# nipponjo/tts-arabic-pytorch

Measured on AMD Instinct MI355X. Metric: audio samples/sec (FastPitch+HiFi-GAN, synthetic 64-phoneme inputs), higher is better.
Workload: dtype f32

## Files before the change

include/ttsamd.h:

```cpp
#ifndef TTSAMD_H
#define TTSAMD_H

#include <stdint.h>

#ifdef __cplusplus
extern "C" {
#endif

#define TTSAMD_OK 0
#define TTSAMD_EINVAL (-1)
#define TTSAMD_EHIP (-2)
#define TTSAMD_ENOMEM (-3)

typedef struct ttsamd_tensor {
    const char* name;
    const float* data;
    int32_t ndim;
    int64_t shape[4];
} ttsamd_tensor;

typedef struct ttsamd_hifigan_cfg {
    int32_t num_mels;
    int32_t upsample_initial_channel;
    int32_t n_ups;
    int32_t upsample_rates[8];
    int32_t upsample_kernel_sizes[8];
    int32_t n_kernels;
    int32_t resblock_kernel_sizes[8];
    int32_t n_dilations;
    int32_t resblock_dilations[8][8];
    int32_t resblock;
} ttsamd_hifigan_cfg;

typedef struct ttsamd_fastpitch_cfg {
    int32_t n_mel_channels;
    int32_t n_symbols;
    int32_t padding_idx;
    int32_t d_model;
    int32_t in_fft_n_layers, in_fft_n_heads, in_fft_d_head, in_fft_kernel, in_fft_filter;
    int32_t out_fft_n_layers, out_fft_n_heads, out_fft_d_head, out_fft_kernel, out_fft_filter;
    int32_t dur_kernel, dur_filter, dur_n_layers;
    int32_t pitch_kernel, pitch_filter, pitch_n_layers, pitch_emb_kernel;
    int32_t energy_conditioning, energy_kernel, energy_filter, energy_n_layers, energy_emb_kernel;
    int32_t n_speakers;
    float speaker_emb_weight;
} ttsamd_fastpitch_cfg;

typedef struct ttsamd_tacotron2_cfg {
    int32_t n_symbol;
    int32_t num_speakers;
    int32_t speaker_embedding_dim;
    int32_t symbol_embedding_dim;
    int32_t encoder_embedding_dim;
    int32_t encoder_n_convolution;
    int32_t encoder_kernel_size;
    int32_t n_mels;
    int32_t prenet_dim;
    int32_t attention_rnn_dim;
    int32_t decoder_rnn_dim;
    int32_t attention_hidden_dim;
    int32_t attention_location_n_filter;
    int32_t attention_location_kernel_size;
    int32_t postnet_n_convolution;
    int32_t postnet_kernel_size;
    int32_t postnet_embedding_dim;
    float gate_threshold;
    int32_t decoder_early_stopping;
} ttsamd_tacotron2_cfg;

typedef struct ttsamd_tagger_cfg {
    int32_t n_vocab;
    int32_t emb_dim;
    int32_t n_lstm;
    int32_t lstm_hidden[4];
    int32_t hard_sigmoid;
    int32_t bn_after_lstm0;
    float bn_eps;
    int32_t n_dense;
    int32_t dense_dim[4];
} ttsamd_tagger_cfg;

const char* ttsamd_last_error(void);
#define TTSAMD_ABI_VERSION 8
int32_t ttsamd_version(void);
int32_t ttsamd_set_option(const char* name, const char* value);
int32_t ttsamd_get_option(const char* name, char* value, int32_t capacity);
const char* ttsamd_option_name(int32_t index);
int32_t ttsamd_options_check(void);
int32_t ttsamd_device_ok(void);


int32_t ttsamd_hifigan_create(const ttsamd_tensor* weights, int32_t n_weights,
                              const ttsamd_hifigan_cfg* cfg, void** handle);
int32_t ttsamd_hifigan_destroy(void* handle);
int64_t ttsamd_hifigan_workspace_bytes(void* handle, int32_t batch, int32_t t_max);
int32_t ttsamd_hifigan_forward(void* handle, const float* mel, const int64_t* lens,
                               int32_t batch, int32_t t_max, float* wave,
                               void* workspace, int64_t workspace_bytes, void* stream);


int32_t ttsamd_fastpitch_create(const ttsamd_tensor* weights, int32_t n_weights,
                                const ttsamd_fastpitch_cfg* cfg, void** handle);
int32_t ttsamd_fastpitch_destroy(void* handle);
int64_t ttsamd_fastpitch_encode_workspace_bytes(void* handle, int32_t batch, int32_t n_tokens);
int64_t ttsamd_fastpitch_decode_workspace_bytes(void* handle, int32_t batch, int32_t t_max);

int32_t ttsamd_fastpitch_encode(void* handle, const int64_t* ids, int32_t batch, int32_t n_tokens,
                                int32_t speaker, float pace, const float* dur_tgt,
                                const float* pitch_tgt, const float* energy_tgt,
                                float pitch_mul, float pitch_add, float max_duration,
                                float* enc_cond, float* dur_pred, float* pitch_pred,
                                float* energy_pred, int64_t* reps, int64_t* dec_lens,
                                void* workspace, int64_t workspace_bytes, void* stream);

int32_t ttsamd_length_regulate(const float* enc, const int64_t* reps, int32_t batch,
                               int32_t n_tokens, int32_t channels, int32_t t_max,
                               float* out, int32_t* idx, void* stream);

int32_t ttsamd_fastpitch_decode(void* handle, float* x, const int64_t* dec_lens, int32_t batch,
                                int32_t t_max, float* mel, void* workspace,
                                int64_t workspace_bytes, void* stream);

int32_t ttsamd_fastpitch_set_batch_mode(void* handle, int32_t mode);

int32_t ttsamd_denoiser_create(void** handle);
int32_t ttsamd_denoiser_destroy(void* handle);
int64_t ttsamd_denoiser_workspace_bytes(int32_t batch, int32_t n_max);
int32_t ttsamd_denoiser_bias_spec(void* handle, const float* audio, const int64_t* n_dev, int32_t n,
                                  float* bias_spec, void* workspace, int64_t workspace_bytes,
                                  void* stream);
int32_t ttsamd_denoise(void* handle, float* wave, int64_t wave_stride, const int64_t* nsamples,
                       int32_t batch, int32_t n_max, const float* bias_spec, float strength,
                       void* workspace, int64_t workspace_bytes, void* stream);

int32_t ttsamd_vocos_create(const ttsamd_tensor* weights, int32_t n_weights, int32_t input_channels,
                            int32_t dim, int32_t intermediate_dim, int32_t num_layers, void** handle);
int32_t ttsamd_vocos_destroy(void* handle);
int64_t ttsamd_vocos_workspace_bytes(void* handle, int32_t batch, int32_t t_max);
int32_t ttsamd_vocos_bias_vec(void* handle, float* bias_vec, void* workspace, int64_t workspace_bytes,
                              void* stream);
int32_t ttsamd_vocos_forward(void* handle, const float* mel, const int64_t* lens, int32_t batch,
                             int32_t t_max, float denoise, const float* bias_vec, float* wave,
                             void* workspace, int64_t workspace_bytes, void* stream);

int32_t ttsamd_vocos_set_padding(void* handle, int32_t mode);

int32_t ttsamd_melspec_create(const float* fbank, int32_t n_mels, int32_t n_fft, int32_t hop_length, int32_t framing,
                              int32_t mag_mode, float log_clip, void** handle);
int32_t ttsamd_melspec_destroy(void* handle);
int32_t ttsamd_melspec_forward(void* handle, const float* wave, int64_t wave_stride, const int64_t* nsamples, int32_t batch,
                               int32_t t_max, float* mel, int64_t* frames_out, void* stream);

#define TTSAMD_OVERSMOOTH_MAX_FRAMES 4096
int32_t ttsamd_cepstral_series(const float* mel, const int64_t* lens, int32_t batch, int32_t n_mels, int32_t t_max, int32_t center,
                               int32_t hann, int32_t q_c, float hqer_scale, float* power, float* series, void* stream);
int32_t ttsamd_cepstral_series_from_power(const float* power, const int64_t* lens, int32_t batch, int32_t n_q, int32_t t_max, int32_t q_c,
                                          int32_t q1, int32_t q2, double eps, double roll_p, float hqer_scale, float* series,
                                          void* stream);
int32_t ttsamd_series_summary(const float* series, const int64_t* lens, int32_t batch, int32_t n_series, int32_t t_max, float* stats,
                              float* feat, void* stream);
int64_t ttsamd_dtw_workspace_bytes(int32_t batch, int32_t ta_max, int32_t tb_max, int32_t channels);
int32_t ttsamd_dtw(const float* a, const int64_t* lens_a, const float* b, const int64_t* lens_b, int32_t batch, int32_t channels,
                   int32_t ta_max, int32_t tb_max, int32_t metric, int32_t window, float* cost, int32_t* path, int32_t* path_len,
                   void* workspace, int64_t workspace_bytes, void* stream);
int32_t ttsamd_dtw_aligned_mae(const float* pred, const float* ref, int32_t batch, int32_t ta_max, int32_t tb_max, const int32_t* path,
                               const int32_t* path_len, float* mae, void* stream);

int32_t ttsamd_tacotron2_create(const ttsamd_tensor* weights, int32_t n_weights,
                                const ttsamd_tacotron2_cfg* cfg, void** handle);
int32_t ttsamd_tacotron2_destroy(void* handle);
int64_t ttsamd_tacotron2_workspace_bytes(void* handle, int32_t batch, int32_t n_tokens, int32_t max_step);
int32_t ttsamd_tacotron2_infer(void* handle, const int64_t* tokens, const int64_t* lengths,
                               const int64_t* speaker_ids, int32_t batch, int32_t n_tokens, int32_t max_step,
                               int64_t dropout_seed, float* mel_post, int32_t* mel_lens, float* alignments,
                               float* mel_raw, int32_t* n_steps, void* workspace, int64_t workspace_bytes,
                               void* stream);

int32_t ttsamd_tagger_create(const ttsamd_tensor* weights, int32_t n_weights, const ttsamd_tagger_cfg* cfg,
                             void** handle);
int32_t ttsamd_tagger_destroy(void* handle);
int64_t ttsamd_tagger_workspace_bytes(void* handle, int32_t batch, int32_t n_chars);
int32_t ttsamd_tagger_forward(void* handle, const int64_t* ids, int32_t batch, int32_t n_chars, float* probs,
                              void* workspace, int64_t workspace_bytes, void* stream);


int64_t ttsamd_conv1d_packed_floats(int32_t cout, int32_t cin, int32_t k);
int32_t ttsamd_conv1d(const float* x, const float* w, const float* bias, const int64_t* lens,
                      int32_t batch, int32_t cin, int32_t cout, int32_t k, int32_t dilation,
                      int32_t lin, float in_slope, int32_t relu_out, float* y, float* packed,
                      void* stream);
int32_t ttsamd_conv1d_ex(const float* x, const float* w, const float* bias, const float* res, const int64_t* lens, int32_t batch,
                         int32_t cin, int32_t cout, int32_t k, int32_t dilation, int32_t lin, float in_slope,
                         int32_t relu_out, int32_t mode, float div, float* y, float* packed, void* stream);

int64_t ttsamd_resblock_pair_packed_floats(int32_t channels, int32_t k, int32_t variant);
int32_t ttsamd_resblock_pair(const float* x, float* y, const float* w1, const float* b1, const float* w2, const float* b2,
                             int32_t channels, int32_t k, int32_t dil, const int64_t* lens, int32_t len_mul, int32_t L,
                             int32_t batch, int32_t mode, float div, float slope, int32_t variant, float* packed, int64_t packed_floats,
                             void* stream);

int64_t ttsamd_resblock2_packed_floats(int32_t channels, int32_t k, int32_t variant);
int32_t ttsamd_resblock2(const float* x, float* y, const float* w1, const float* b1, const float* w2, const float* b2, int32_t channels,
                         int32_t k, int32_t dil1, int32_t dil2, const int64_t* lens, int32_t len_mul, int32_t L, int32_t batch, int32_t mode,
                         float div, float slope, int32_t variant, float* packed, int64_t packed_floats, void* stream);

int32_t ttsamd_bfo_pack(const float* x, int32_t batch, int32_t channels, int32_t len, float slope, void* out, void* stream);
int32_t ttsamd_bfo_unpack(const void* in, int32_t batch, int32_t channels, int32_t len, float slope, float* out, void* stream);
int64_t ttsamd_bfo_weight_elems(int32_t cout, int32_t cin, int32_t k, int32_t up);
int32_t ttsamd_bfo_pack_weight(const float* w, int32_t cout, int32_t cin, int32_t k, int32_t up, uint16_t* out);
int32_t ttsamd_bfo_conv1d(const void* x, const void* w_packed, const float* bias, const void* res, const void* sum_in,
                          const int64_t* lens, int32_t len_mul, int32_t batch, int32_t cin, int32_t cout, int32_t k,
                          int32_t dilation, int32_t up, int32_t len_in, int32_t mode, float div, float res_slope,
                          float out_slope, void* y, float* y_f32, const float* res_f32, void* stream);
int32_t ttsamd_bfo_resblock_pair(const void* x, const void* w1, const float* b1, const void* w2, const float* b2,
                                 const void* sum_in, const int64_t* lens, int32_t len_mul, int32_t batch, int32_t channels,
                                 int32_t k, int32_t dilation, int32_t len, int32_t mode, float div, float in_slope,
                                 float mid_slope, float out_slope, void* y, void* stream);
int32_t ttsamd_bfo_resblock_chain(const void* x, const void* const* w1, const float* const* b1, const void* const* w2,
                                  const float* const* b2, const int32_t* dilations, const void* sum_in, const int64_t* lens,
                                  int32_t len_mul, int32_t batch, int32_t channels, int32_t len, int32_t mode, float div,
                                  float in_slope, float mid_slope, float out_slope, void* y, void* stream, int32_t k);
int32_t ttsamd_bfo_conv_post(const void* x, const float* w, const float* bias, const int64_t* lens, int32_t len_mul,
                             int32_t batch, int32_t channels, int32_t len, float* wave, int64_t wave_stride, void* stream);

int32_t ttsamd_bfo3_pack(const float* x, int32_t batch, int32_t channels, int32_t len, float slope, void* out, void* stream);
int32_t ttsamd_bfo3_unpack(const void* in, int32_t batch, int32_t channels, int32_t len, float slope, float* out, void* stream);
int64_t ttsamd_bfo3_weight_elems(int32_t cout, int32_t cin, int32_t k, int32_t up);
int32_t ttsamd_bfo3_pack_weight(const float* w, int32_t cout, int32_t cin, int32_t k, int32_t up, uint16_t* out);
int32_t ttsamd_bfo3_conv1d(const void* x, const void* w_packed, const float* bias, const void* res, const void* sum_in,
                           const int64_t* lens, int32_t len_mul, int32_t batch, int32_t cin, int32_t cout, int32_t k,
                           int32_t dilation, int32_t up, int32_t len_in, int32_t mode, float div, float res_slope,
                           float out_slope, void* y, float* y_f32, const float* res_f32, void* stream);
int32_t ttsamd_bfo3_resblock_pair(const void* x, const void* w1, const float* b1, const void* w2, const float* b2,
                                  const void* sum_in, const int64_t* lens, int32_t len_mul, int32_t batch, int32_t channels,
                                  int32_t k, int32_t dilation, int32_t len, int32_t mode, float div, float in_slope,
                                  float mid_slope, float out_slope, void* y, void* stream);
int32_t ttsamd_bfo3_resblock_chain(const void* x, const void* const* w1, const float* const* b1, const void* const* w2,
                                   const float* const* b2, const int32_t* dilations, const void* sum_in, const int64_t* lens,
                                   int32_t len_mul, int32_t batch, int32_t channels, int32_t len, int32_t mode, float div,
                                   float in_slope, float mid_slope, float out_slope, void* y, void* stream);
int32_t ttsamd_bfo3_conv_post(const void* x, const float* w, const float* bias, const int64_t* lens, int32_t len_mul,
                              int32_t batch, int32_t channels, int32_t len, float* wave, int64_t wave_stride, void* stream);

int32_t ttsamd_set_precision(int32_t precision);
int32_t ttsamd_get_precision(void);

#define TTSAMD_DP_ID_BYTES 128
#define TTSAMD_DP_HIFIGAN 0
#define TTSAMD_DP_FASTPITCH 1
int32_t ttsamd_dp_unique_id(void* id128 );
int32_t ttsamd_dp_init(int32_t rank, int32_t world, const void* id128 , void** comm);
int32_t ttsamd_dp_destroy(void* comm);
int32_t ttsamd_dp_rank(void* comm);
int32_t ttsamd_dp_world(void* comm);
int32_t ttsamd_dp_broadcast(void* comm, void* buf, int64_t nbytes, int32_t root, void* stream);
int32_t ttsamd_dp_broadcast_weights(void* comm, int32_t kind, void* handle, int32_t root, void* stream);
int32_t ttsamd_dp_allgather(void* comm, const void* send, void* recv, int64_t nbytes_per_rank, void* stream);
int32_t ttsamd_dp_pack_audio(const float* wave, int64_t wave_stride, const int64_t* nsamples, int32_t batch,
                             int64_t n_max, float* packed, void* stream);
int32_t ttsamd_dp_gather_audio(void* comm, const float* packed, float* recv, const int64_t* counts,
                               const int64_t* offsets, int32_t root, void* stream);

int32_t ttsamd_profile_enable(int32_t on);
int32_t ttsamd_profile_read(double* out3);

#ifdef __cplusplus
}
#endif
#endif
```

tts-arabic-pytorch_amd/csrc/api.hip:

```cpp
#include <cerrno>
#include <cstdio>
#include <cstdlib>
#include <cstring>
#include <algorithm>
#include <atomic>
#include <mutex>
#include <string>
#include <vector>

#include "kernels.hpp"

namespace ttsamd {

static thread_local std::string g_err;

void set_error(const char* fmt, ...) {
    char buf[1024];
    va_list ap;
    va_start(ap, fmt);
    vsnprintf(buf, sizeof(buf), fmt, ap);
    va_end(ap);
    g_err = buf;
}

static int g_precision = 0;
int32_t default_precision() { return g_precision; }

struct Prof {
    std::mutex mu;
    bool on = false;
    std::vector<hipEvent_t> ev;
    size_t used = 0;
    size_t launches = 0;
    double flops_per_frame = 0.0;
} g_prof;

void prof_section_begin(hipStream_t s) {
    if (!g_prof.on) return;
    std::lock_guard<std::mutex> lk(g_prof.mu);
    if (g_prof.used + 2 > g_prof.ev.size()) {
        hipEvent_t a, b;
        if (hipEventCreate(&a) != hipSuccess || hipEventCreate(&b) != hipSuccess) return;
        g_prof.ev.push_back(a);
        g_prof.ev.push_back(b);
    }
    (void)hipEventRecord(g_prof.ev[g_prof.used], s);
}

void prof_section_end(hipStream_t s) {
    if (!g_prof.on) return;
    std::lock_guard<std::mutex> lk(g_prof.mu);
    if (g_prof.used + 2 > g_prof.ev.size()) return;
    (void)hipEventRecord(g_prof.ev[g_prof.used + 1], s);
    g_prof.used += 2;
}

void prof_add(double flops_per_frame) {
    if (!g_prof.on) return;
    std::lock_guard<std::mutex> lk(g_prof.mu);
    g_prof.launches += 1;
    g_prof.flops_per_frame += flops_per_frame;
}

void prof_begin(hipStream_t s, double flops_per_frame) {
    prof_section_begin(s);
    prof_add(flops_per_frame);
}

void prof_end(hipStream_t s) { prof_section_end(s); }

struct HifiGan;
struct FastPitch;
struct Denoiser;
struct Vocos;
int32_t vocos_create(const ttsamd_tensor*, int32_t, int32_t, int32_t, int32_t, int32_t, Vocos**);
void vocos_destroy(Vocos*);
int64_t vocos_workspace_bytes(const Vocos*, int32_t, int32_t);
int64_t vocos_bias_workspace_bytes(const Vocos*);
int32_t vocos_bias_vec(const Vocos*, float*, void*, int64_t, hipStream_t);
int32_t vocos_forward(const Vocos*, const float*, const int64_t*, int32_t, int32_t, float, const float*, float*, void*,
                      int64_t, hipStream_t);
int32_t vocos_set_padding(Vocos*, int32_t);
struct MelSpec;
int32_t melspec_create(const float*, int32_t, int32_t, int32_t, int32_t, int32_t, float, MelSpec**);
void melspec_destroy(MelSpec*);
int32_t melspec_forward(const MelSpec*, const float*, int64_t, const int64_t*, int32_t, int32_t, float*, int64_t*, hipStream_t);
int32_t cepstral_series(const float*, const int64_t*, int32_t, int32_t, int32_t, int32_t, int32_t, int32_t, float, float*, float*, hipStream_t);
int32_t cepstral_series_from_power(const float*, const int64_t*, int32_t, int32_t, int32_t, int32_t, int32_t, int32_t, double, double, float,
                                   float*, hipStream_t);
int32_t series_summary(const float*, const int64_t*, int32_t, int32_t, int32_t, float*, float*, hipStream_t);
int64_t dtw_workspace_bytes(int32_t, int32_t, int32_t, int32_t);
int32_t dtw(const float*, const int64_t*, const float*, const int64_t*, int32_t, int32_t, int32_t, int32_t, int32_t, int32_t, float*,
            int32_t*, int32_t*, void*, int64_t, hipStream_t);
int32_t dtw_aligned_mae(const float*, const float*, int32_t, int32_t, int32_t, const int32_t*, const int32_t*, float*, hipStream_t);
struct Taco2;
int32_t tacotron2_create(const ttsamd_tensor*, int32_t, const ttsamd_tacotron2_cfg*, Taco2**);
void tacotron2_destroy(Taco2*);
int64_t tacotron2_workspace_bytes(const Taco2*, int32_t, int32_t, int32_t);
int32_t tacotron2_infer(const Taco2*, const int64_t*, const int64_t*, const int64_t*, int32_t, int32_t, int32_t, int64_t,
                        float*, int32_t*, float*, float*, int32_t*, void*, int64_t, hipStream_t);
struct Tagger;
int32_t tagger_create(const ttsamd_tensor*, int32_t, const ttsamd_tagger_cfg*, Tagger**);
void tagger_destroy(Tagger*);
int64_t tagger_workspace_bytes(const Tagger*, int32_t, int32_t);
int32_t tagger_forward(const Tagger*, const int64_t*, int32_t, int32_t, float*, void*, int64_t, hipStream_t);
int32_t denoiser_create(Denoiser**);
void denoiser_destroy(Denoiser*);
int64_t denoiser_workspace_bytes(int32_t, int32_t);
int32_t denoiser_bias_spec(const Denoiser*, const float*, const int64_t*, int32_t, float*, void*, int64_t, hipStream_t);
int32_t denoise(const Denoiser*, float*, int64_t, const int64_t*, int32_t, int32_t, const float*, float, void*, int64_t,
                hipStream_t);
int32_t hifigan_create(const ttsamd_tensor*, int32_t, const ttsamd_hifigan_cfg*, HifiGan**);
void hifigan_destroy(HifiGan*);
int64_t hifigan_workspace_bytes(const HifiGan*, int32_t, int32_t);
int32_t hifigan_forward(const HifiGan*, const float*, const int64_t*, int32_t, int32_t, float*, void*, int64_t,
                        hipStream_t);
int32_t fastpitch_create(const ttsamd_tensor*, int32_t, const ttsamd_fastpitch_cfg*, int32_t, FastPitch**);
void fastpitch_destroy(FastPitch*);
int64_t fastpitch_encode_workspace_bytes(const FastPitch*, int32_t, int32_t);
int64_t fastpitch_decode_workspace_bytes(const FastPitch*, int32_t, int32_t);
int32_t fastpitch_encode(const FastPitch*, const int64_t*, int32_t, int32_t, int32_t, float, const float*,
                         const float*, const float*, float, float, float, float*, float*, float*, float*, int64_t*,
                         int64_t*, void*, int64_t, hipStream_t);
void fastpitch_set_batch_mode(const FastPitch*, int);
int32_t fastpitch_decode(const FastPitch*, float*, const int64_t*, int32_t, int32_t, float*, void*, int64_t,
                         hipStream_t);

__global__ void pack_conv_weight_kernel(const float* __restrict__ w, int cout, int cin, int k, int cp,
                                        float* __restrict__ out) {
    const int64_t i = (int64_t)blockIdx.x * 256 + threadIdx.x;
    const int64_t n = (int64_t)cin * k * cp;
    if (i >= n) return;
    const int pq = (int)(i % 4);
    const int co = (int)((i / 4) % cp);
    const int kk = (int)((i / (4 * (int64_t)cp)) % 2);
    const int t = (int)((i / (8 * (int64_t)cp)) % k);
    const int o = (int)(i / (8 * (int64_t)cp * k));
    out[i] = co < cout ? w[((int64_t)co * cin + (8 * o + 2 * pq + kk)) * k + t] : 0.f;
}

__global__ void split_bf16_kernel(const float* __restrict__ packed, int64_t n, unsigned short* __restrict__ out) {
    const int64_t i = (int64_t)blockIdx.x * 256 + threadIdx.x;
    if (i >= n) return;
    const float f = packed[i];
    unsigned u = __float_as_uint(f);
    u += 0x7fffu + ((u >> 16) & 1u);
    const unsigned h = u >> 16;
    const float r = f - __uint_as_float(h << 16);
    unsigned v = __float_as_uint(r);
    v += 0x7fffu + ((v >> 16) & 1u);
    out[i] = (unsigned short)h;
    out[n + i] = (unsigned short)(v >> 16);
}

namespace {
struct OptDesc { const char* name; int kind; long long lo, hi; };
const OptDesc kOpts[OPT_COUNT] = {
#define TTS_OPT_DESC(name, kind, lo, hi) {"TTSAMD_" #name, kind, lo, hi},
    TTS_OPTIONS(TTS_OPT_DESC)
#undef TTS_OPT_DESC
};
std::atomic<const char*> g_opt[OPT_COUNT];
std::once_flag g_opt_once;
std::string g_opt_env_error;

bool opt_valid(const OptDesc& d, const char* v) {
    if (!v || !*v) return false;
    char* end = nullptr;
    errno = 0;
    const long long x = std::strtoll(v, &end, d.kind == 1 ? 16 : 10);
    return errno == 0 && end != v && *end == '\0' && x >= d.lo && x <= d.hi;
}
void opt_init() {
    std::call_once(g_opt_once, [] {
        for (int i = 0; i < OPT_COUNT; ++i) {
            const char* e = std::getenv(kOpts[i].name);
            if (!e || !*e) continue;
            if (!opt_valid(kOpts[i], e)) {
                if (g_opt_env_error.empty()) {
                    char buf[256];
                    std::snprintf(buf, sizeof buf, "%s='%s' in the environment is not a valid value (%s in [%llx, %llx])", kOpts[i].name, e,
                                  kOpts[i].kind == 1 ? "hex mask" : "integer", kOpts[i].lo, kOpts[i].hi);
                    g_opt_env_error = buf;
                }
                continue;
            }
            g_opt[i].store(strdup(e), std::memory_order_release);
        }
    });
}
int opt_find(const char* name) {
    if (!name) return -1;
    for (int i = 0; i < OPT_COUNT; ++i)
        if (std::strcmp(name, kOpts[i].name) == 0 || std::strcmp(name, kOpts[i].name + 7) == 0) return i;
    return -1;
}
}

int64_t opt_int(Opt o, int64_t unset) {
    opt_init();
    const char* v = g_opt[o].load(std::memory_order_acquire);
    return v ? (int64_t)std::strtoll(v, nullptr, kOpts[o].kind == 1 ? 16 : 10) : unset;
}

}

using namespace ttsamd;

extern "C" {

const char* ttsamd_last_error(void) { return g_err.c_str(); }
int32_t ttsamd_version(void) { return TTSAMD_ABI_VERSION; }

int32_t ttsamd_set_option(const char* name, const char* value) {
    opt_init();
    const int i = opt_find(name);
    TTS_REQUIRE(i >= 0, "set_option: unknown option '%s' (ttsamd_option_name lists them)", name ? name : "(null)");
    if (!value || !*value) {
        g_opt[i].store(nullptr, std::memory_order_release);
        return 0;
    }
    TTS_REQUIRE(opt_valid(kOpts[i], value), "set_option: %s='%s' is not a valid value (%s in [%llx, %llx])", kOpts[i].name, value,
                kOpts[i].kind == 1 ? "hex mask" : "integer", kOpts[i].lo, kOpts[i].hi);
    g_opt[i].store(strdup(value), std::memory_order_release);
    return 0;
}
int32_t ttsamd_get_option(const char* name, char* value, int32_t capacity) {
    opt_init();
    const int i = opt_find(name);
    TTS_REQUIRE(i >= 0 && value && capacity > 0, "get_option: unknown option '%s' or no buffer", name ? name : "(null)");
    const char* v = g_opt[i].load(std::memory_order_acquire);
    std::snprintf(value, (size_t)capacity, "%s", v ? v : "");
    return 0;
}
const char* ttsamd_option_name(int32_t index) { return (index >= 0 && index < OPT_COUNT) ? kOpts[index].name : nullptr; }
int32_t ttsamd_options_check(void) {
    opt_init();
    TTS_REQUIRE(g_opt_env_error.empty(), "%s", g_opt_env_error.c_str());
    return 0;
}

int32_t ttsamd_device_ok(void) {
    int n = 0;
    if (hipGetDeviceCount(&n) != hipSuccess || n <= 0) return 0;
    hipDeviceProp_t prop;
    if (hipGetDeviceProperties(&prop, 0) != hipSuccess) return 0;
    return std::string(prop.gcnArchName).rfind("gfx950", 0) == 0 ? 1 : 0;
}

int32_t ttsamd_hifigan_create(const ttsamd_tensor* weights, int32_t n, const ttsamd_hifigan_cfg* cfg, void** handle) {
    HifiGan* h = nullptr;
    const int32_t rc = hifigan_create(weights, n, cfg, &h);
    if (rc == 0) *handle = h;
    return rc;
}
int32_t ttsamd_hifigan_destroy(void* handle) {
    hifigan_destroy((HifiGan*)handle);
    return 0;
}
int64_t ttsamd_hifigan_workspace_bytes(void* handle, int32_t batch, int32_t t_max) {
    if (!handle || batch < 1 || t_max < 1) return 0;
    return hifigan_workspace_bytes((HifiGan*)handle, batch, t_max);
}
int32_t ttsamd_hifigan_forward(void* handle, const float* mel, const int64_t* lens, int32_t batch, int32_t t_max,
                               float* wave, void* workspace, int64_t workspace_bytes, void* stream) {
    return hifigan_forward((HifiGan*)handle, mel, lens, batch, t_max, wave, workspace, workspace_bytes,
                           (hipStream_t)stream);
}

int32_t ttsamd_fastpitch_create(const ttsamd_tensor* weights, int32_t n, const ttsamd_fastpitch_cfg* cfg,
                                void** handle) {
    FastPitch* h = nullptr;
    const int32_t rc = fastpitch_create(weights, n, cfg, 16384, &h);
    if (rc == 0) *handle = h;
    return rc;
}
int32_t ttsamd_fastpitch_destroy(void* handle) {
    fastpitch_destroy((FastPitch*)handle);
    return 0;
}
int64_t ttsamd_fastpitch_encode_workspace_bytes(void* handle, int32_t batch, int32_t n_tokens) {
    if (!handle || batch < 1 || n_tokens < 1) return 0;
    return fastpitch_encode_workspace_bytes((FastPitch*)handle, batch, n_tokens);
}
int64_t ttsamd_fastpitch_decode_workspace_bytes(void* handle, int32_t batch, int32_t t_max) {
    if (!handle || batch < 1 || t_max < 1) return 0;
    return fastpitch_decode_workspace_bytes((FastPitch*)handle, batch, t_max);
}
int32_t ttsamd_fastpitch_encode(void* handle, const int64_t* ids, int32_t batch, int32_t n_tokens, int32_t speaker,
                                float pace, const float* dur_tgt, const float* pitch_tgt, const float* energy_tgt,
                                float pitch_mul, float pitch_add, float max_duration, float* enc_cond,
                                float* dur_pred, float* pitch_pred, float* energy_pred, int64_t* reps,
                                int64_t* dec_lens, void* workspace, int64_t workspace_bytes, void* stream) {
    return fastpitch_encode((FastPitch*)handle, ids, batch, n_tokens, speaker, pace, dur_tgt, pitch_tgt, energy_tgt,
                            pitch_mul, pitch_add, max_duration, enc_cond, dur_pred, pitch_pred, energy_pred, reps,
                            dec_lens, workspace, workspace_bytes, (hipStream_t)stream);
}
int32_t ttsamd_length_regulate(const float* enc, const int64_t* reps, int32_t batch, int32_t n_tokens,
                               int32_t channels, int32_t t_max, float* out, int32_t* idx, void* stream) {
    TTS_REQUIRE(enc && reps && out && batch >= 1 && n_tokens >= 1 && channels >= 1 && t_max >= 0,
                "length_regulate: bad argument");
    return launch_regulate_gather(enc, reps, nullptr, 0, batch, n_tokens, channels, t_max, out, idx,
                                  (hipStream_t)stream);
}
int32_t ttsamd_fastpitch_set_batch_mode(void* handle, int32_t mode) {
    TTS_REQUIRE(handle != nullptr, "fastpitch_set_batch_mode: null handle");
    TTS_REQUIRE(mode == 0 || mode == 1, "fastpitch_set_batch_mode: mode %d (0 = padded-batch arithmetic, 1 = every utterance alone)", mode);
    fastpitch_set_batch_mode((const FastPitch*)handle, mode);
    return 0;
}
int32_t ttsamd_fastpitch_decode(void* handle, float* x, const int64_t* dec_lens, int32_t batch, int32_t t_max,
                                float* mel, void* workspace, int64_t workspace_bytes, void* stream) {
    return fastpitch_decode((FastPitch*)handle, x, dec_lens, batch, t_max, mel, workspace, workspace_bytes,
                            (hipStream_t)stream);
}

int32_t ttsamd_denoiser_create(void** handle) {
    Denoiser* h = nullptr;
    const int32_t rc = denoiser_create(&h);
    if (rc == 0) *handle = h;
    return rc;
}
int32_t ttsamd_denoiser_destroy(void* handle) {
    denoiser_destroy((Denoiser*)handle);
    return 0;
}
int64_t ttsamd_denoiser_workspace_bytes(int32_t batch, int32_t n_max) {
    if (batch < 1 || n_max < 1) return 0;
    return denoiser_workspace_bytes(batch, n_max);
}
int32_t ttsamd_denoiser_bias_spec(void* handle, const float* audio, const int64_t* n_dev, int32_t n,
                                  float* bias_spec, void* workspace, int64_t workspace_bytes, void* stream) {
    return denoiser_bias_spec((Denoiser*)handle, audio, n_dev, n, bias_spec, workspace, workspace_bytes,
                              (hipStream_t)stream);
}
int32_t ttsamd_denoise(void* handle, float* wave, int64_t wave_stride, const int64_t* nsamples, int32_t batch,
                       int32_t n_max, const float* bias_spec, float strength, void* workspace,
                       int64_t workspace_bytes, void* stream) {
    return denoise((Denoiser*)handle, wave, wave_stride, nsamples, batch, n_max, bias_spec, strength, workspace,
                   workspace_bytes, (hipStream_t)stream);
}

int32_t ttsamd_vocos_create(const ttsamd_tensor* weights, int32_t n, int32_t input_channels, int32_t dim,
                            int32_t intermediate_dim, int32_t num_layers, void** handle) {
    Vocos* h = nullptr;
    const int32_t rc = vocos_create(weights, n, input_channels, dim, intermediate_dim, num_layers, &h);
    if (rc == 0) *handle = h;
    return rc;
}
int32_t ttsamd_vocos_destroy(void* handle) {
    vocos_destroy((Vocos*)handle);
    return 0;
}
int64_t ttsamd_vocos_workspace_bytes(void* handle, int32_t batch, int32_t t_max) {
    if (!handle || batch < 1 || t_max < 1) return 0;
    const int64_t a = vocos_workspace_bytes((Vocos*)handle, batch, t_max), b = vocos_bias_workspace_bytes((Vocos*)handle);
    return a > b ? a : b;
}
int32_t ttsamd_vocos_bias_vec(void* handle, float* bias_vec, void* workspace, int64_t workspace_bytes, void* stream) {
    return vocos_bias_vec((Vocos*)handle, bias_vec, workspace, workspace_bytes, (hipStream_t)stream);
}
int32_t ttsamd_vocos_forward(void* handle, const float* mel, const int64_t* lens, int32_t batch, int32_t t_max,
                             float denoise, const float* bias_vec, float* wave, void* workspace,
                             int64_t workspace_bytes, void* stream) {
    return vocos_forward((Vocos*)handle, mel, lens, batch, t_max, denoise, bias_vec, wave, workspace, workspace_bytes,
                         (hipStream_t)stream);
}

int32_t ttsamd_vocos_set_padding(void* handle, int32_t mode) { return vocos_set_padding((Vocos*)handle, mode); }

int32_t ttsamd_melspec_create(const float* fbank, int32_t n_mels, int32_t n_fft, int32_t hop_length, int32_t framing,
                              int32_t mag_mode, float log_clip, void** handle) {
    TTS_REQUIRE(handle, "melspec_create: null handle");
    MelSpec* h = nullptr;
    const int32_t rc = melspec_create(fbank, n_mels, n_fft, hop_length, framing, mag_mode, log_clip, &h);
    if (rc == 0) *handle = h;
    return rc;
}
int32_t ttsamd_melspec_destroy(void* handle) {
    melspec_destroy((MelSpec*)handle);
    return 0;
}
int32_t ttsamd_melspec_forward(void* handle, const float* wave, int64_t wave_stride, const int64_t* nsamples, int32_t batch,
                               int32_t t_max, float* mel, int64_t* frames_out, void* stream) {
    return melspec_forward((const MelSpec*)handle, wave, wave_stride, nsamples, batch, t_max, mel, frames_out, (hipStream_t)stream);
}

int32_t ttsamd_cepstral_series(const float* mel, const int64_t* lens, int32_t batch, int32_t n_mels, int32_t t_max, int32_t center,
                               int32_t hann, int32_t q_c, float hqer_scale, float* power, float* series, void* stream) {
    return cepstral_series(mel, lens, batch, n_mels, t_max, center, hann, q_c, hqer_scale, power, series, (hipStream_t)stream);
}
int32_t ttsamd_cepstral_series_from_power(const float* power, const int64_t* lens, int32_t batch, int32_t n_q, int32_t t_max, int32_t q_c,
                                          int32_t q1, int32_t q2, double eps, double roll_p, float hqer_scale, float* series,
                                          void* stream) {
    return cepstral_series_from_power(power, lens, batch, n_q, t_max, q_c, q1, q2, eps, roll_p, hqer_scale, series, (hipStream_t)stream);
}
int32_t ttsamd_series_summary(const float* series, const int64_t* lens, int32_t batch, int32_t n_series, int32_t t_max, float* stats,
                              float* feat, void* stream) {
    return series_summary(series, lens, batch, n_series, t_max, stats, feat, (hipStream_t)stream);
}
int64_t ttsamd_dtw_workspace_bytes(int32_t batch, int32_t ta_max, int32_t tb_max, int32_t channels) {
    return dtw_workspace_bytes(batch, ta_max, tb_max, channels);
}
int32_t ttsamd_dtw(const float* a, const int64_t* lens_a, const float* b, const int64_t* lens_b, int32_t batch, int32_t channels,
                   int32_t ta_max, int32_t tb_max, int32_t metric, int32_t window, float* cost, int32_t* path, int32_t* path_len,
                   void* workspace, int64_t workspace_bytes, void* stream) {
    return dtw(a, lens_a, b, lens_b, batch, channels, ta_max, tb_max, metric, window, cost, path, path_len, workspace, workspace_bytes,
               (hipStream_t)stream);
}
int32_t ttsamd_dtw_aligned_mae(const float* pred, const float* ref, int32_t batch, int32_t ta_max, int32_t tb_max, const int32_t* path,
                               const int32_t* path_len, float* mae, void* stream) {
    return dtw_aligned_mae(pred, ref, batch, ta_max, tb_max, path, path_len, mae, (hipStream_t)stream);
}

int32_t ttsamd_tacotron2_create(const ttsamd_tensor* weights, int32_t n, const ttsamd_tacotron2_cfg* cfg, void** handle) {
    TTS_REQUIRE(handle, "tacotron2_create: null handle");
    Taco2* h = nullptr;
    const int32_t rc = tacotron2_create(weights, n, cfg, &h);
    if (rc == 0) *handle = h;
    return rc;
}
int32_t ttsamd_tacotron2_destroy(void* handle) {
    tacotron2_destroy((Taco2*)handle);
    return 0;
}
int64_t ttsamd_tacotron2_workspace_bytes(void* handle, int32_t batch, int32_t n_tokens, int32_t max_step) {
    if (!handle || batch < 1 || n_tokens < 1 || max_step < 1) return 0;
    return tacotron2_workspace_bytes((Taco2*)handle, batch, n_tokens, max_step);
}
int32_t ttsamd_tacotron2_infer(void* handle, const int64_t* tokens, const int64_t* lengths, const int64_t* speaker_ids,
                               int32_t batch, int32_t n_tokens, int32_t max_step, int64_t dropout_seed, float* mel_post,
                               int32_t* mel_lens, float* alignments, float* mel_raw, int32_t* n_steps, void* workspace,
                               int64_t workspace_bytes, void* stream) {
    return tacotron2_infer((Taco2*)handle, tokens, lengths, speaker_ids, batch, n_tokens, max_step, dropout_seed, mel_post,
                           mel_lens, alignments, mel_raw, n_steps, workspace, workspace_bytes, (hipStream_t)stream);
}

int32_t ttsamd_tagger_create(const ttsamd_tensor* weights, int32_t n, const ttsamd_tagger_cfg* cfg, void** handle) {
    TTS_REQUIRE(handle, "tagger_create: null handle");
    Tagger* h = nullptr;
    const int32_t rc = tagger_create(weights, n, cfg, &h);
    if (rc == 0) *handle = h;
    return rc;
}
int32_t ttsamd_tagger_destroy(void* handle) {
    tagger_destroy((Tagger*)handle);
    return 0;
}
int64_t ttsamd_tagger_workspace_bytes(void* handle, int32_t batch, int32_t n_chars) {
    if (!handle || batch < 1 || n_chars < 1) return 0;
    return tagger_workspace_bytes((Tagger*)handle, batch, n_chars);
}
int32_t ttsamd_tagger_forward(void* handle, const int64_t* ids, int32_t batch, int32_t n_chars, float* probs,
                              void* workspace, int64_t workspace_bytes, void* stream) {
    return tagger_forward((Tagger*)handle, ids, batch, n_chars, probs, workspace, workspace_bytes, (hipStream_t)stream);
}

int64_t ttsamd_conv1d_packed_floats(int32_t cout, int32_t cin, int32_t k) {
    return 2 * (int64_t)cin * k * cout_padded(cout) +
           ((k == 3 || k == 7 || k == 11) ? (int64_t)cin * (wino2_groups(k) + wino4_groups(k)) * cout_padded(cout) : 0);
}

__global__ void pack_wino4_weight_kernel(const float* __restrict__ w, int cout, int cin, int k, int cp, float* __restrict__ out) {
    const int ng = k == 3 ? 6 : (k == 7 ? 16 : 24), nsf = k == 3 ? 1 : (k == 7 ? 2 : 4);
    const int64_t i = (int64_t)blockIdx.x * 256 + threadIdx.x;
    const int64_t n = (int64_t)cin * ng * cp;
    if (i >= n) return;
    const int pq = (int)(i & 3);
    const int64_t r = i >> 2;
    const int co = (int)(r % cp);
    const int64_t r2 = r / cp;
    const int kk = (int)(r2 & 1);
    const int64_t r3 = r2 >> 1;
    const int t = (int)(r3 % ng), o = (int)(r3 / ng);
    float v = 0.f;
    if (co < cout) {
        const float* g = w + ((int64_t)co * cin + (8 * o + 2 * pq + kk)) * k;
        if (t < 6 * nsf) {
            const int s = t / 6, j = t % 6;
            const double g0 = g[3 * s], g1 = 3 * s + 1 < k ? g[3 * s + 1] : 0.0, g2 = 3 * s + 2 < k ? g[3 * s + 2] : 0.0;
            v = j == 0 ? (float)(g0 / 4) : (j == 1 ? (float)(-(g0 + g1 + g2) / 6) : (j == 2 ? (float)(-(g0 - g1 + g2) / 6) :
                (j == 3 ? (float)(g0 / 24 + g1 / 12 + g2 / 6) : (j == 4 ? (float)(g0 / 24 - g1 / 12 + g2 / 6) : (float)g2))));
        } else {
            v = g[6];
        }
    }
    out[i] = v;
}

__global__ void pack_wino2_weight_kernel(const float* __restrict__ w, int cout, int cin, int k, int cp, float* __restrict__ out) {
    const int ns = k / 3, ng = 4 * ns + 2 * (k - 3 * ns);
    const int64_t i = (int64_t)blockIdx.x * 256 + threadIdx.x;
    const int64_t n = (int64_t)cin * ng * cp;
    if (i >= n) return;
    const int pq = (int)(i & 3);
    const int64_t r = i >> 2;
    const int co = (int)(r % cp);
    const int64_t r2 = r / cp;
    const int kk = (int)(r2 & 1);
    const int64_t r3 = r2 >> 1;
    const int t = (int)(r3 % ng), o = (int)(r3 / ng);
    float v = 0.f;
    if (co < cout) {
        const float* g = w + ((int64_t)co * cin + (8 * o + 2 * pq + kk)) * k;
        if (t < 4 * ns) {
            const int s = t >> 2, j = t & 3;
            const double g0 = g[3 * s], g1 = g[3 * s + 1], g2 = g[3 * s + 2];
            v = j == 0 ? (float)g0 : (j == 1 ? (float)((g0 + g1 + g2) * 0.5) : (j == 2 ? (float)((g0 - g1 + g2) * 0.5) : (float)g2));
        } else {
            const int l = (t - 4 * ns) >> 1;
            v = ((t - 4 * ns) & 1) ? -g[3 * ns + l] : g[3 * ns + l];
        }
    }
    out[i] = v;
}

int32_t ttsamd_conv1d_ex(const float* x, const float* w, const float* bias, const float* res, const int64_t* lens, int32_t batch,
                         int32_t cin, int32_t cout, int32_t k, int32_t dilation, int32_t lin, float in_slope,
                         int32_t relu_out, int32_t mode, float div, float* y, float* packed, void* stream) {
    TTS_REQUIRE(x && w && y && packed, "conv1d: null argument");
    TTS_REQUIRE(mode >= 0 && mode <= 2 && (mode != 2 || div != 0.f), "conv1d: bad mode / div");
    TTS_REQUIRE(relu_out == 0 || mode == 0, "conv1d: relu_out with an accumulate mode (mode %d) is not defined", mode);
    hipStream_t s = (hipStream_t)stream;
    const int cp = cout_padded(cout);
    const int64_t n = (int64_t)cin * k * cp;
    hipLaunchKernelGGL(pack_conv_weight_kernel, dim3((unsigned)((n + 255) / 256)), dim3(256), 0, s, w, cout, cin, k,
                       cp, packed);
    TTS_CHECK_HIP(hipGetLastError());
    ConvParams p;
    std::memset(&p, 0, sizeof(p));
    p.x = x; p.x_bs = (int64_t)cin * lin; p.x_cs = lin;
    p.w = packed; p.bias = bias;
    p.precision = default_precision();
    if (p.precision != 0) {
        unsigned short* planes = reinterpret_cast<unsigned short*>(packed + n);
        hipLaunchKernelGGL(split_bf16_kernel, dim3((unsigned)((n + 255) / 256)), dim3(256), 0, s, packed, n, planes);
        TTS_CHECK_HIP(hipGetLastError());
        p.w_bf16 = planes;
    }
    if ((k == 3 || k == 7 || k == 11) && p.precision == 0 && cin % 8 == 0) {
        float* wino = packed + 2 * n;
        const int64_t nw = (int64_t)cin * wino2_groups(k) * cp;
        hipLaunchKernelGGL(pack_wino2_weight_kernel, dim3((unsigned)((nw + 255) / 256)), dim3(256), 0, s, w, cout, cin, k, cp, wino);
        TTS_CHECK_HIP(hipGetLastError());
        p.w_wino = wino;
        float* wino4 = wino + nw;
        const int64_t nw4 = (int64_t)cin * wino4_groups(k) * cp;
        hipLaunchKernelGGL(pack_wino4_weight_kernel, dim3((unsigned)((nw4 + 255) / 256)), dim3(256), 0, s, w, cout, cin, k, cp, wino4);
        TTS_CHECK_HIP(hipGetLastError());
        p.w_wino4 = wino4;
    }
    p.y = y; p.y_bs = (int64_t)cout * lin; p.y_cs = lin; p.y_ts = 1;
    p.lens_in = lens; p.lens_out = lens; p.len_in_mul = 1; p.len_out_mul = 1;
    p.Lin = lin; p.Nout = lin; p.Cin = cin; p.Cout = cout; p.CoutP = cp; p.K = k;
    p.dil = dilation; p.pad = (k * dilation - dilation) / 2;
    p.res = res; p.r_bs = (int64_t)cout * lin; p.r_cs = lin;
    p.n_phase = 1; p.in_slope = in_slope; p.relu_out = relu_out; p.mode = mode; p.div = div; p.batch = batch;
    prof_begin(s, 2.0 * cout * cin * k);
    const int32_t rc = launch_conv(p, s);
    prof_end(s);
    return rc;
}

int32_t ttsamd_conv1d(const float* x, const float* w, const float* bias, const int64_t* lens, int32_t batch,
                      int32_t cin, int32_t cout, int32_t k, int32_t dilation, int32_t lin, float in_slope,
                      int32_t relu_out, float* y, float* packed, void* stream) {
    return ttsamd_conv1d_ex(x, w, bias, nullptr, lens, batch, cin, cout, k, dilation, lin, in_slope, relu_out, 0, 1.f, y, packed, stream);
}

int64_t ttsamd_resblock_pair_packed_floats(int32_t channels, int32_t k, int32_t variant) {
    if (channels < 1 || k < 1) return 0;
    const int64_t n = 2 * (int64_t)channels * k * channels;
    const int nwino = (variant == 4 ? 1 : (variant == 5 ? 2 : 0));
    if (variant == 6) return n + ((k == 3 || k == 7 || k == 11) ? 2 * (int64_t)channels * wino4_groups(k) * channels : 0);
    return n + ((k == 3 || k == 7 || k == 11) ? nwino * (int64_t)channels * wino2_groups(k) * channels : 0);
}

int32_t ttsamd_resblock_pair(const float* x, float* y, const float* w1, const float* b1, const float* w2, const float* b2,
                             int32_t channels, int32_t k, int32_t dil, const int64_t* lens, int32_t len_mul, int32_t L,
                             int32_t batch, int32_t mode, float div, float slope, int32_t variant, float* packed, int64_t packed_floats,
                             void* stream) {
    TTS_REQUIRE(x && y && w1 && b1 && w2 && b2 && packed && channels % 32 == 0 && k >= 1 && batch >= 1 && L >= 1 && len_mul >= 1 &&
                mode >= 0 && mode <= 2, "resblock_pair: bad argument");
    TTS_REQUIRE(packed_floats >= ttsamd_resblock_pair_packed_floats(channels, k, variant),
                "resblock_pair: `packed` holds %lld floats, variant %d at C = %d, k = %d needs %lld (ttsamd_resblock_pair_packed_floats)",
                (long long)packed_floats, variant, channels, k, (long long)ttsamd_resblock_pair_packed_floats(channels, k, variant));
    hipStream_t s = (hipStream_t)stream;
    const int64_t n = (int64_t)channels * k * channels;
    for (int i = 0; i < 2; ++i) {
        hipLaunchKernelGGL(pack_conv_weight_kernel, dim3((unsigned)((n + 255) / 256)), dim3(256), 0, s, i == 0 ? w1 : w2, channels,
                           channels, k, channels, packed + i * n);
        TTS_CHECK_HIP(hipGetLastError());
    }
    const double fl = 2.0 * (2.0 * channels * channels * k);
    int32_t rc;
    prof_begin(s, fl);
    if (variant == 1) {
        rc = launch_fused_pair(channels, x, y, packed, b1, packed + n, b2, k, dil, lens, len_mul, L, batch, mode, div, slope, s);
    } else if (variant >= 2 && variant <= 5) {
        const float *w2w = nullptr, *w1w = nullptr;
        if (variant >= 4) {
            TTS_REQUIRE((k == 3 || k == 7 || k == 11) && (channels <= 64 || (variant == 5 && channels == 128)),
                        "resblock_pair: variants 4 / 5 are built for C = 32 / 64 (5: and 128), k = 3 / 7 / 11");
            const int64_t nw = (int64_t)channels * wino2_groups(k) * channels;
            for (int i = 0; i < (variant == 5 ? 2 : 1); ++i) {
                float* wino = packed + 2 * n + i * nw;
                hipLaunchKernelGGL(pack_wino2_weight_kernel, dim3((unsigned)((nw + 255) / 256)), dim3(256), 0, s, i == 0 ? w2 : w1, channels,
                                   channels, k, channels, wino);
                TTS_CHECK_HIP(hipGetLastError());
                (i == 0 ? w2w : w1w) = wino;
            }
        }
        rc = launch_fused_pair2(channels, x, y, packed, b1, packed + n, b2, k, dil, lens, len_mul, L, batch, mode, div, slope,
                                variant == 3 ? 1 : 2, s, w2w, w1w);
    } else if (variant == 6) {
        TTS_REQUIRE(channels == 32 && (k == 3 || k == 7 || k == 11), "resblock_pair: variant 6 is built for C = 32, k = 3 / 7 / 11");
        const int64_t nw4 = (int64_t)channels * wino4_groups(k) * channels;
        for (int i = 0; i < 2; ++i) {
            hipLaunchKernelGGL(pack_wino4_weight_kernel, dim3((unsigned)((nw4 + 255) / 256)), dim3(256), 0, s, i == 0 ? w1 : w2, channels,
                               channels, k, channels, packed + 2 * n + i * nw4);
            TTS_CHECK_HIP(hipGetLastError());
        }
        rc = launch_fused_pair4(channels, x, y, packed + 2 * n, b1, packed + 2 * n + nw4, b2, k, dil, lens, len_mul, L, batch, mode, div,
                                slope, s);
    } else if (variant == -1) {
        rc = 0;
    } else {
        set_error("resblock_pair: variant %d (1: first generation, 2 / 3: second generation with 256- / 128-column blocks, 4 / 5: 256 columns + Winograd phase B / both phases, 6: C = 32 with both phases on Winograd F(4,3))", variant);
        rc = TTSAMD_EINVAL;
    }
    prof_end(s);
    return rc;
}

int64_t ttsamd_resblock2_packed_floats(int32_t channels, int32_t k, int32_t variant) {
    if (channels < 1 || k < 1 || (variant != 1 && variant != 2)) return 0;
    return 2 * (int64_t)channels * k * channels;
}

int32_t ttsamd_resblock2(const float* x, float* y, const float* w1, const float* b1, const float* w2, const float* b2, int32_t channels,
                         int32_t k, int32_t dil1, int32_t dil2, const int64_t* lens, int32_t len_mul, int32_t L, int32_t batch, int32_t mode,
                         float div, float slope, int32_t variant, float* packed, int64_t packed_floats, void* stream) {
    TTS_REQUIRE(x && y && w1 && b1 && w2 && b2 && packed && channels % 32 == 0 && channels >= 32 && k >= 1 && batch >= 1 && L >= 1 &&
                len_mul >= 1 && mode >= 0 && mode <= 2 && x != y, "resblock2: bad argument");
    TTS_REQUIRE(variant == 1 || variant == 2, "resblock2: variant %d (1: two single-conv launches, 2: both convs in one launch)", variant);
    TTS_REQUIRE(packed_floats >= ttsamd_resblock2_packed_floats(channels, k, variant),
                "resblock2: `packed` holds %lld floats, C = %d, k = %d needs %lld (ttsamd_resblock2_packed_floats)", (long long)packed_floats,
                channels, k, (long long)ttsamd_resblock2_packed_floats(channels, k, variant));
    if (variant == 1) {
        TTS_REQUIRE(resblock2_conv_supported(channels, k, dil1, L, x, y) && resblock2_conv_supported(channels, k, dil2, L, x, y),
                    "resblock2: variant 1 does not cover C = %d, k = %d, dilations %d / %d (C = 32 / 64 / 128, k = 3 / 5 / 7 / 11, "
                    "dilation 1..16)", channels, k, dil1, dil2);
    } else {
        TTS_REQUIRE(resblock2_pair_supported(channels, k, dil1, dil2, L, x, y),
                    "resblock2: variant 2 does not cover C = %d, k = %d, dilations %d / %d (C = 32 / 64, k = 3 / 5 / 7 / 11, dilation "
                    "1..16, (k - 1) * dil2 <= 256)", channels, k, dil1, dil2);
    }
    hipStream_t s = (hipStream_t)stream;
    const int64_t n = (int64_t)channels * k * channels;
    for (int i = 0; i < 2; ++i) {
        hipLaunchKernelGGL(pack_conv_weight_kernel, dim3((unsigned)((n + 255) / 256)), dim3(256), 0, s, i == 0 ? w1 : w2, channels,
                           channels, k, channels, packed + i * n);
        TTS_CHECK_HIP(hipGetLastError());
    }
    prof_begin(s, 2.0 * (2.0 * channels * channels * k));
    int32_t rc;
    if (variant == 2) {
        rc = launch_resblock2_pair(channels, x, y, packed, b1, packed + n, b2, k, dil1, dil2, lens, len_mul, L, batch, mode, div, slope, s);
    } else {
        float* x1 = nullptr;
        TTS_CHECK_HIP(hipMallocAsync((void**)&x1, (size_t)batch * channels * L * sizeof(float), s));
        rc = launch_resblock2_conv(channels, x, x1, packed, b1, k, dil1, lens, len_mul, L, batch, 0, 1.f, slope, s);
        if (rc == 0) rc = launch_resblock2_conv(channels, x1, y, packed + n, b2, k, dil2, lens, len_mul, L, batch, mode, div, slope, s);
        const hipError_t e = hipFreeAsync(x1, s);
        if (rc == 0 && e != hipSuccess) {
            set_error("resblock2: hipFreeAsync failed: %s", hipGetErrorString(e));
            rc = TTSAMD_EHIP;
        }
    }
    prof_end(s);
    return rc;
}

int32_t ttsamd_set_precision(int32_t precision) {
    TTS_REQUIRE(precision >= 0 && precision <= 2, "set_precision: 0 = fp32 MFMA, 1 = bf16 MFMA, 2 = split-bf16 MFMA");
    g_precision = precision;
    return 0;
}
int32_t ttsamd_get_precision(void) { return g_precision; }

int32_t ttsamd_profile_enable(int32_t on) {
    std::lock_guard<std::mutex> lk(g_prof.mu);
    g_prof.on = on != 0;
    g_prof.used = 0;
    g_prof.launches = 0;
    g_prof.flops_per_frame = 0.0;
    return 0;
}

int32_t ttsamd_profile_read(double* out3) {
    TTS_REQUIRE(out3, "profile_read: null argument");
    std::lock_guard<std::mutex> lk(g_prof.mu);
    std::vector<std::pair<float, float>> iv;
    for (size_t i = 0; i + 1 < g_prof.used; i += 2) {
        TTS_CHECK_HIP(hipEventSynchronize(g_prof.ev[i + 1]));
        float t0 = 0.f, t1 = 0.f;
        if (i > 0) TTS_CHECK_HIP(hipEventElapsedTime(&t0, g_prof.ev[0], g_prof.ev[i]));
        TTS_CHECK_HIP(hipEventElapsedTime(&t1, g_prof.ev[0], g_prof.ev[i + 1]));
        iv.emplace_back(t0, std::max(t0, t1));
    }
    std::sort(iv.begin(), iv.end());
    double ms = 0.0;
    float lo = 0.f, hi = -1.f;
    for (const auto& v : iv) {
        if (hi < lo || v.first > hi) {
            if (hi >= lo) ms += hi - lo;
            lo = v.first;
            hi = v.second;
        } else {
            hi = std::max(hi, v.second);
        }
    }
    if (hi >= lo) ms += hi - lo;
    out3[0] = ms;
    out3[1] = (double)g_prof.launches;
    out3[2] = (double)(g_prof.used / 2);
    return 0;
}

}
```

tts-arabic-pytorch_amd/csrc/common.hpp:

```cpp
#pragma once
#include <hip/hip_runtime.h>
#include <stdint.h>
#include <atomic>
#include <cstdarg>
#include <cstdio>
#include <cstdlib>
#include <string>

#include "../../include/ttsamd.h"

namespace ttsamd {

void set_error(const char* fmt, ...);

#define TTS_CHECK_HIP(expr)                                                         \
    do {                                                                            \
        hipError_t e_ = (expr);                                                     \
        if (e_ != hipSuccess) {                                                     \
            ttsamd::set_error("%s failed: %s (%s:%d)", #expr, hipGetErrorString(e_), \
                              __FILE__, __LINE__);                                  \
            return TTSAMD_EHIP;                                                     \
        }                                                                           \
    } while (0)

#define TTS_REQUIRE(cond, ...)              \
    do {                                    \
        if (!(cond)) {                      \
            ttsamd::set_error(__VA_ARGS__); \
            return TTSAMD_EINVAL;           \
        }                                   \
    } while (0)

#define TTS_TRY(expr)               \
    do {                            \
        int32_t rc_ = (expr);       \
        if (rc_ != 0) return rc_;   \
    } while (0)

inline int64_t align_up(int64_t x, int64_t a) { return (x + a - 1) / a * a; }

inline hipError_t lds_opt_in(const void* fn, int bytes, std::atomic<uint64_t>& done) {
    int dev = 0;
    hipError_t e = hipGetDevice(&dev);
    if (e != hipSuccess) return e;
    if (dev >= 0 && dev < 64 && ((done.load(std::memory_order_acquire) >> dev) & 1)) return hipSuccess;
    e = hipFuncSetAttribute(fn, hipFuncAttributeMaxDynamicSharedMemorySize, bytes);
    if (e == hipSuccess && dev >= 0 && dev < 64) done.fetch_or(1ull << dev, std::memory_order_release);
    return e;
}

#define TTS_OPTIONS(X)                                                                                     \
    X(HIFIGAN_STREAMS, 0, 0, 1)    \
    X(WINO, 0, 0, 1)                                              \
    X(WINO2, 0, 0, 31)             \
    X(WINO4, 0, 0, 31)             \
    X(FUSED_PAIR, 0, 0, 1)                   \
    X(FUSED2, 0, 0, 1)                                           \
    X(FUSED2_MASK, 1, 0, 0x1ff)               \
    X(FUSED2_MASK_N1, 1, 0, 0x1ff)          \
    X(FUSED2_WB, 0, 0, 2)                     \
    X(PAIR4, 0, 0, 1)              \
    X(CONVT, 0, 0, 1)                              \
    X(BFO, 0, 0, 1)                \
    X(BFO_CHAIN, 0, 0, 1)                           \
    X(BFO_CHAIN7, 0, 0, 1)                                 \
    X(BFO_FF, 0, 0, 1)                              \
    X(BFO_SPLITK, 0, 0, 1)                                              \
    X(BFO_SMALL_TILES, 0, 0, 1)            \
    X(BF16_ATTN, 0, 0, 1)                                         \
    X(BF16_PACKED_T, 0, 0, 1)                   \
    X(ATT_RA, 0, 1, 4)                             \
    X(ATT_SPLIT, 0, 0, 1)                      \
    X(XCD_W, 0, 0, 1)                            \
    X(XCD_WMAX_KB, 0, 0, 1 << 20)     \
    X(DEEP_SPLITK, 0, 0, 1)        \
    X(TACO_PERSISTENT, 0, 0, 2)    \
    X(TACO_SEG, 0, 8, 1 << 20)     \
    X(RESBLOCK2_PAIR, 1, 0, 0x3f)
enum Opt : int {
#define TTS_OPT_ENUM(name, kind, lo, hi) OPT_##name,
    TTS_OPTIONS(TTS_OPT_ENUM)
#undef TTS_OPT_ENUM
    OPT_COUNT
};
int64_t opt_int(Opt o, int64_t unset);

struct Arena {
    char* base;
    int64_t size;
    int64_t off = 0;
    bool ok = true;
    Arena(void* p, int64_t n) : base((char*)p), size(n) {}
    template <typename T>
    T* take(int64_t count) {
        int64_t bytes = align_up(count * (int64_t)sizeof(T), 256);
        if (base != nullptr && off + bytes > size) ok = false;
        T* r = base ? (T*)(base + off) : nullptr;
        off += bytes;
        return r;
    }
};

struct ConvParams {
    const float* x;
    int64_t x_bs;
    int32_t x_cs;
    const float* w;
    const void* w_bf16;
    const float* w_wino;
    const float* w_wino4;
    int32_t precision;
    const float* bias;
    float* y;
    int64_t y_bs;
    int32_t y_cs, y_ts;
    const float* res;
    int64_t r_bs;
    int32_t r_cs;
    const int64_t* lens_in;
    const int64_t* lens_out;
    int32_t len_in_mul, len_out_mul;
    int32_t Lin, Nout;
    int32_t Cin, Cout, CoutP, K;
    int32_t dil, pad;
    int32_t n_phase;
    int32_t phase_p;
    float in_slope;
    const float* scale;
    int32_t relu_out;
    int32_t mode;
    float div;
    int32_t batch;
    float* splitk_ws;
    int64_t splitk_floats;
    int32_t ksplit;
    int32_t y_packed;
    float pack_slope;
    int32_t x_packed;
    int32_t xcd_w;
    int32_t tile_major;
    int32_t compact;
    unsigned long long* timing;
};
constexpr int64_t kSplitKFloats = 4 << 20;
constexpr int64_t kSplitKFloatsFp = 8 << 20;

void conv_log(const char* kind, int K, int cin, int cout, int nout, int batch, int has_res, int mode, int len_mul, int ragged,
              int n_phase);
bool compact_order(const void* lens, int batch);
int32_t launch_conv(const ConvParams& p, hipStream_t stream);
bool convt_supported(const ConvParams& p);
int32_t launch_convt(const ConvParams& p, hipStream_t stream);
bool fused_pair_supported(int32_t channels, int32_t k, int32_t dil, int32_t L, const float* x, const float* y);
int32_t launch_fused_pair(int32_t channels, const float* x, float* y, const float* w1, const float* b1, const float* w2,
                          const float* b2, int32_t k, int32_t dil, const int64_t* lens, int32_t len_mul, int32_t L, int32_t batch,
                          int32_t mode, float div, float slope, hipStream_t stream);
bool fused_pair2_supported(int32_t channels, int32_t k, int32_t dil, int32_t L, const float* x, const float* y, int32_t ntw);
int32_t launch_fused_pair2(int32_t channels, const float* x, float* y, const float* w1, const float* b1, const float* w2,
                           const float* b2, int32_t k, int32_t dil, const int64_t* lens, int32_t len_mul, int32_t L, int32_t batch,
                           int32_t mode, float div, float slope, int32_t ntw, hipStream_t stream, const float* w2_wino = nullptr,
                           const float* w1_wino = nullptr);
bool fused_pair4_supported(int32_t channels, int32_t k, int32_t dil, int32_t L, const float* x, const float* y);
int32_t launch_fused_pair4(int32_t channels, const float* x, float* y, const float* w1_wino4, const float* b1, const float* w2_wino4,
                           const float* b2, int32_t k, int32_t dil, const int64_t* lens, int32_t len_mul, int32_t L, int32_t batch,
                           int32_t mode, float div, float slope, hipStream_t stream);
bool resblock2_conv_supported(int32_t channels, int32_t k, int32_t dil, int32_t L, const float* x, const float* y);
int32_t launch_resblock2_conv(int32_t channels, const float* x, float* y, const float* w, const float* b, int32_t k, int32_t dil,
                              const int64_t* lens, int32_t len_mul, int32_t L, int32_t batch, int32_t mode, float div, float slope,
                              hipStream_t stream);
bool resblock2_pair_supported(int32_t channels, int32_t k, int32_t d1, int32_t d2, int32_t L, const float* x, const float* y);
int32_t launch_resblock2_pair(int32_t channels, const float* x, float* y, const float* w1, const float* b1, const float* w2,
                              const float* b2, int32_t k, int32_t d1, int32_t d2, const int64_t* lens, int32_t len_mul, int32_t L,
                              int32_t batch, int32_t mode, float div, float slope, hipStream_t stream);
int wino_route(const ConvParams& p);
int32_t launch_wino(const ConvParams& p, hipStream_t stream);
void pack_wino_weight(const float* w, int cout, int cin, float* out);
int wino2_groups(int k);
int wino2_block_outputs(int coutp, int dil);
int32_t launch_wino2(const ConvParams& p, hipStream_t stream);
void pack_wino2_weight(const float* w, int cout, int cin, int k, float* out);
int wino4_groups(int k);
int wino4_block_outputs(int dil);
int wino4_ksplit(const ConvParams& p);
int32_t launch_splitk_reduce(const ConvParams& q, hipStream_t stream);
int32_t launch_wino4(const ConvParams& p, hipStream_t stream);
void wino4_filter_groups(const float* g, int k, float* o);
void pack_wino4_weight(const float* w, int cout, int cin, int k, float* out);
void pack_conv_weight(const float* w, int cout, int cin, int k, float* out);
void pack_convt_weight(const float* w, int cin, int cout, int kt, int u, int p, float* out);
inline int cout_padded(int cout) { return (int)align_up(cout, 32); }
void split_packed_bf16(const float* packed, int64_t n, uint16_t* out);
int32_t default_precision();

#ifdef __HIPCC__
__device__ __forceinline__ bool live_tile(const int64_t* __restrict__ lens, const int mul, const int n_max, const int tile_w,
                                          const int batch, const unsigned lin, int& b, int& tile) {
    const int lane = threadIdx.x & 63;
    unsigned base = 0;
    for (int u0 = 0; u0 < batch; u0 += 64) {
        int n = 0;
        if (u0 + lane < batch) n = (max(min(n_max, (int)lens[u0 + lane] * mul), 0) + tile_w - 1) / tile_w;
        int incl = n;
#pragma unroll
        for (int d = 1; d < 64; d <<= 1) {
            const int t = __shfl_up(incl, d, 64);
            if (lane >= d) incl += t;
        }
        const unsigned total = (unsigned)__shfl(incl, 63, 64);
        if (lin < base + total) {
            const unsigned long long m = __ballot(base + (unsigned)incl > lin);
            const int l = __ffsll((long long)m) - 1;
            b = u0 + l;
            tile = (int)(lin - base) - (__shfl(incl, l, 64) - __shfl(n, l, 64));
            return true;
        }
        base += total;
    }
    return false;
}
#endif

}
```

tts-arabic-pytorch_amd/csrc/conv_wino4.hip:

```cpp
#include <cstdlib>
#include <cstring>

#include <algorithm>
#include <vector>

#include "conv_mfma_common.hpp"
#include "bfo.hpp"

namespace ttsamd {

typedef float w4_f32x4 __attribute__((ext_vector_type(4)));
typedef float w4_f32x2 __attribute__((ext_vector_type(2)));

template <int K, int NOCT_, int NSTAGE_, int EPI_ = 0>
struct Wino4Geo {
    static constexpr int WM = 2, WN = 2;
    static constexpr int NSF = K == 1 ? 0 : (K == 3 ? 1 : (K == 7 ? 2 : 4));
    static constexpr int NL = (K == 7 || K == 1) ? 1 : 0;
    static constexpr int NG = K == 1 ? 4 : (K == 3 ? 6 : (K == 7 ? 16 : 23));
    static constexpr int NGQ = (NG + 1) & ~1;
    static constexpr bool WSHARE = K == 1;
    static constexpr int NGW = WSHARE ? 1 : NGQ;
    static constexpr int NPL = (NL || EPI_ == 3) ? 8 : 6;
    static constexpr int NPOS = K == 1 ? 4 : (K == 3 ? 6 : (K == 7 ? 10 : 14));
    static constexpr int NOCT = NOCT_, NSTAGE = NSTAGE_;
    static constexpr int NPH = K == 11 ? 2 : 1;
    static constexpr int NGPM = NPH == 1 ? NG : 12;
    static constexpr int CO_BLK = WM * 32;
    static constexpr int NTUP = WN * 32;
    static constexpr int NT_BLK = 4 * NTUP;
    static constexpr int BUF4 = NOCT * 2 * NGPM * NTUP;
    static constexpr int PF = 4;
    static constexpr int NM = 4;
    __host__ __device__ static constexpr int glo(int ph) { return NPH == 1 ? 0 : 12 * ph; }
    __host__ __device__ static constexpr int ngp(int ph) { return NPH == 1 ? NG : (ph == 0 ? 12 : NG - 12); }
    __host__ __device__ static constexpr int ngq(int ph) { return NPH == 1 ? NGQ : 12; }
    __host__ __device__ static constexpr int gfirst(int g) { return g < 6 * NSF ? 3 * (g / 6) : 3 * NSF + (g - 6 * NSF); }
    __host__ __device__ static constexpr int glast(int g) {
        return g < 6 * NSF ? (3 * (g / 6) + 5 < NPOS ? 3 * (g / 6) + 5 : NPOS - 1) : 3 * NSF + (g - 6 * NSF);
    }
    __host__ __device__ static constexpr int plane(int g) {
        return g < 6 * NSF ? g % 6 : ((g - 6 * NSF) == 0 ? 0 : ((g - 6 * NSF) == 1 ? 6 : ((g - 6 * NSF) == 2 ? 7 : 5)));
    }
    __host__ __device__ static constexpr int mlo(int ph) { return gfirst(glo(ph)); }
    __host__ __device__ static constexpr int mhi(int ph) {
        int m = 0;
        for (int g = glo(ph); g < glo(ph) + ngp(ph); ++g) m = glast(g) > m ? glast(g) : m;
        return m;
    }
    __host__ __device__ static constexpr int npos(int ph) { return mhi(ph) - mlo(ph) + 1; }
    static constexpr int NPOSP = npos(0) > npos(NPH - 1) ? npos(0) : npos(NPH - 1);
    __host__ __device__ static constexpr int ngap(int ph) { return NOCT * ngp(ph) * NM; }
    __host__ __device__ static constexpr int nwj(int ph) { return NOCT * ngp(ph); }
    __host__ __device__ static constexpr int fdiv4(int e) { return e >= 0 ? e / 4 : -((3 - e) / 4); }
    __host__ __device__ static constexpr int vlo(int ph) { return fdiv4(mlo(ph) - (K - 1) / 2); }
    __host__ __device__ static constexpr int nvec(int ph) { return fdiv4(mhi(ph) - (K - 1) / 2) - vlo(ph) + 1; }
    static constexpr int NVP = nvec(0) > nvec(NPH - 1) ? nvec(0) : nvec(NPH - 1);
    __host__ __device__ static constexpr int nljv(int ph) { return NOCT * 2 * nvec(ph); }
    static constexpr int DAV = (K == 3 || K == 1) ? 8 : 16;
    __host__ __device__ static constexpr int tw0v(int ph) { return DAV + 2 * nljv(ph); }
    __host__ __device__ static constexpr int wsv(int ph) { return (ngap(ph) - tw0v(ph)) / nwj(ph); }
    static_assert(wsv(0) >= 1 && wsv(NPH - 1) >= 1, "one write job per gap at most (vector loads)");
    static constexpr int RAWW = 320;
    static constexpr int NROW = 2 * NOCT;
    static constexpr int RAW_BYTES = 4 * (NROW * RAWW * 4 + 16);
    static constexpr int DAT = K == 7 ? 16 : (K == 11 ? 12 : 8);
    __host__ __device__ static constexpr int nrj(int ph) { return NROW * ((npos(ph) + 1) / 2); }
    __host__ __device__ static constexpr bool loads_in(int ph) { return ph == 0; }
    __host__ __device__ static constexpr int tr_r0(int ph) { return loads_in(ph) ? DAT + 2 * NROW : 0; }
    __host__ __device__ static constexpr int tw0t(int ph) { return tr_r0(ph) + nrj(ph) + 1; }
    __host__ __device__ static constexpr int wst(int ph) { return (ngap(ph) - tw0t(ph)) / nwj(ph); }
    static_assert(wst(0) >= 1 && wst(NPH - 1) >= 1, "one write job per gap at most (strip path)");
    static_assert((WSHARE ? NOCT : NOCT * ngq(0)) % PF == 0 && (NOCT * ngq(NPH - 1)) % PF == 0, "queue slots line up across steps");
    static_assert((size_t)NSTAGE * BUF4 * 16 <= 80 * 1024, "two blocks per CU");
    static_assert(NPH == 1 || NOCT == 1, "phases split an octet's groups");
};

__device__ __host__ constexpr int wino4_tile(int d, int ntup) { return (4 * ntup / (4 * d)) * (4 * d); }

template <int K, int NOCT_, int NSTAGE_, int EPI, int LP>
__global__ __launch_bounds__(256, kConvMinWaves) void conv1d_wino4_f32(const ConvParams p) {
    extern __shared__ __attribute__((aligned(16))) float4 smem4[];
    using G = Wino4Geo<K, NOCT_, NSTAGE_, EPI>;
    constexpr int WN = G::WN, NSF = G::NSF, NOCT = G::NOCT, NSTAGE = G::NSTAGE, NPL = G::NPL, NGPM = G::NGPM;
    constexpr int CO_BLK = G::CO_BLK, NTUP = G::NTUP, NT_BLK = G::NT_BLK, PF = G::PF;
    constexpr int NPH = G::NPH, NPOSP = G::NPOSP, NM = G::NM;
    constexpr bool D1 = LP == 1, TR = LP == 2;
    static_assert(D1 || TR, "window path");
    const int dil = D1 ? 1 : p.dil;
    const int nt_eff = wino4_tile(dil, NTUP), ntup_eff = nt_eff / 4;
    const int tiles_y = p.CoutP / CO_BLK;
    const int per_tile = tiles_y * p.ksplit;
    const unsigned sidx = blockIdx.x, xcd = sidx & 7u, u = sidx >> 3;
    const int yk = (int)(u % (unsigned)per_tile);
    const unsigned gt = (u / (unsigned)per_tile) * 8u + xcd;
    const int n_tiles_x = (p.Nout + nt_eff - 1) / nt_eff;
    int b = (int)(gt / (unsigned)n_tiles_x);
    int q0 = (int)(gt % (unsigned)n_tiles_x) * nt_eff;
    if (p.compact) {
        int tile = 0;
        if (!live_tile(p.lens_out, p.len_out_mul, p.Nout, nt_eff, p.batch, gt, b, tile)) return;
        b = __builtin_amdgcn_readfirstlane(b);
        q0 = __builtin_amdgcn_readfirstlane(tile) * nt_eff;
    } else if (b >= p.batch) {
        return;
    }
    const int tid = threadIdx.x, lane = tid & 63, wid = tid >> 6;
    const int wm = wid / WN, wn = wid % WN;
    const int ks = yk / tiles_y;
    const int co_blk0 = (yk - ks * tiles_y) * CO_BLK;
    int n_out = p.Nout;
    if (p.lens_out) n_out = min(n_out, (int)p.lens_out[b] * p.len_out_mul);
    if (q0 >= n_out) return;
    int in_len = p.Lin;
    if (p.lens_in) in_len = min(in_len, (int)p.lens_in[b] * p.len_in_mul);

    const int x_cs = p.x_cs, CoutP = p.CoutP;
    const int chunks_all = p.Cin / (8 * NOCT);
    const int c_beg = (int)((int64_t)ks * chunks_all / p.ksplit), n_chunks = (int)((int64_t)(ks + 1) * chunks_all / p.ksplit);
    const int n_groups = (p.Cin / 8) * G::NGW;
    const float* __restrict__ xb = p.x + (int64_t)b * p.x_bs;
    const float in_slope = p.in_slope;

    float ep_bias = 0.f;
    if (tid < CO_BLK && p.bias) ep_bias = p.bias[min(co_blk0 + tid, p.Cout - 1)];

    const int kk = lane >> 5, l31 = lane & 31;
    const int pe = wn * 32 + l31;
    const int col_e = dil == 1 ? 4 * pe : (pe / dil) * 4 * dil + pe % dil;
    f32x16 acc[NPL];
#pragma unroll
    for (int g = 0; g < NPL; ++g)
#pragma unroll
        for (int r = 0; r < 16; ++r) acc[g][r] = 0.f;
    constexpr bool preload = EPI == 3;
    if constexpr (preload) {
        const int wm_s = __builtin_amdgcn_readfirstlane(wm);
        const int row0 = co_blk0 + wm_s * 32;
        const int qv = q0 + col_e;
        const int voff = (qv < n_out ? qv : 0) * 4;
        {
            const int r_cs = p.r_cs;
            const bfo_i4 rs = bfo_rsrc(p.res + (int64_t)b * p.r_bs, (unsigned)p.Cout * (unsigned)r_cs * 4u);
            const int vk = 4 * kk * r_cs * 4;
#pragma unroll
            for (int r = 0; r < 16; ++r) {
                const w4_f32x4 t = __builtin_bit_cast(w4_f32x4, bfo_ld16(rs, voff + vk, (row0 + (r & 3) + 8 * (r >> 2)) * r_cs * 4, 0));
                acc[0][r] = t.x; acc[6][r] = t.y; acc[7][r] = t.z; acc[5][r] = t.w;
            }
        }
        if (p.mode != 0) {
            const int y_cs_ = p.y_cs;
            const bfo_i4 ys = bfo_rsrc(p.y + (int64_t)b * p.y_bs, (unsigned)p.Cout * (unsigned)y_cs_ * 4u);
            const int vk = 4 * kk * y_cs_ * 4;
#pragma unroll
            for (int r = 0; r < 16; ++r) {
                const w4_f32x4 t = __builtin_bit_cast(w4_f32x4, bfo_ld16(ys, voff + vk, (row0 + (r & 3) + 8 * (r >> 2)) * y_cs_ * 4, 0));
                acc[0][r] += t.x; acc[6][r] += t.y; acc[7][r] += t.z; acc[5][r] += t.w;
            }
        }
    }

    const bfo_i4 wrs = bfo_rsrc(K == 1 ? p.w : p.w_wino4, (unsigned)n_groups * 2u * (unsigned)CoutP * 16u);
    const int wv = (kk * CoutP + co_blk0 + wm * 32 + l31) * 16;
    const int wstep = 2 * CoutP * 16, wlast = (n_groups - 1) * wstep;
    int wso = c_beg * NOCT * G::NGW * wstep;
    w4_f32x4 aq[PF];
#pragma unroll
    for (int g = 0; g < PF; ++g) {
        aq[g] = __builtin_bit_cast(w4_f32x4, bfo_ld16(wrs, wv, wso, 0));
        wso = min(wso + wstep, wlast);
    }

    const int sh = __builtin_amdgcn_readfirstlane((tid >> 7) & 1), skk = __builtin_amdgcn_readfirstlane((tid >> 6) & 1);
    w4_f32x2 sx[D1 ? 1 : NOCT][D1 ? 1 : NPOSP];
    w4_f32x4 sv[D1 ? NOCT : 1][2][D1 ? G::NVP : 1];
    w4_f32x2 ta[NOCT], tb[NOCT];
    const int spe = min(lane, ntup_eff - 1);
    const int xw0 = (q0 + 4 * lane) * 4;
    constexpr int pad_c = (K - 1) / 2;
    const int ch_off = (4 * sh + skk) * x_cs;

#define TTS_VJOB_IDX(PH, J)                                                                          \
        const int nv_ = G::nvec(PH);                                                                 \
        const int ol_ = (J) / (2 * nv_), pp_ = ((J) / nv_) % 2, vi_ = (J) % nv_;
#define TTS_VLOAD_JOB(PH, J, XSO)                                                                    \
    {                                                                                                \
        TTS_VJOB_IDX(PH, J)                                                                          \
        const bfo_i4 xrs_ = bfo_rsrc(xb + ((XSO) + ch_off + (8 * ol_ + 2 * pp_) * x_cs), (unsigned)in_len * 4u);     \
        sv[ol_][pp_][vi_] = __builtin_bit_cast(w4_f32x4, bfo_ld16(xrs_, xw0 + 16 * (G::vlo(PH) + vi_), 0, 0));      \
    }
#define TTS_VACT_JOB(PH, A)                                                                          \
    {                                                                                                \
        TTS_VJOB_IDX(PH, (A) / 2)                                                                    \
        if ((A) % 2 == 0) {                                                                          \
            sv[ol_][pp_][vi_].x = bfo_lrelu(sv[ol_][pp_][vi_].x, in_slope);                          \
            sv[ol_][pp_][vi_].y = bfo_lrelu(sv[ol_][pp_][vi_].y, in_slope);                          \
        } else {                                                                                     \
            sv[ol_][pp_][vi_].z = bfo_lrelu(sv[ol_][pp_][vi_].z, in_slope);                          \
            sv[ol_][pp_][vi_].w = bfo_lrelu(sv[ol_][pp_][vi_].w, in_slope);                          \
        }                                                                                            \
    }
    float* const strip = reinterpret_cast<float*>(smem4 + NSTAGE * G::BUF4) + wid * (G::NROW * G::RAWW + 4);
    const int tr_a = (q0 - pad_c * dil) & ~3;
    const int tr_off = q0 + (dil == 1 ? 4 * spe : (spe / dil) * 4 * dil + spe % dil) - pad_c * dil - tr_a;
    w4_f32x4 rv[TR ? G::NROW : 1][2];
#define TTS_TLOAD_JOB(J, XSO)                                                                        \
    {                                                                                                \
        const int pp_ = (J) / 2, vs_ = (J) % 2;                                                      \
        const bfo_i4 xrs_ = bfo_rsrc(xb + ((XSO) + ch_off + (8 * (pp_ / 2) + 2 * (pp_ % 2)) * x_cs), (unsigned)in_len * 4u); \
        const int v_ = lane + 64 * vs_;                                                              \
        rv[pp_][vs_] = __builtin_bit_cast(w4_f32x4, bfo_ld16(xrs_, (vs_ == 1 && lane >= 16) ? BFO_OOB : (tr_a + 4 * v_) * 4, 0, 0)); \
    }
#define TTS_TSTORE_JOB(J)                                                                            \
    {                                                                                                \
        const int pp_ = (J) / 2, vs_ = (J) % 2;                                                      \
        w4_f32x4 a_ = rv[pp_][vs_];                                                                  \
        a_.x = bfo_lrelu(a_.x, in_slope); a_.y = bfo_lrelu(a_.y, in_slope);                          \
        a_.z = bfo_lrelu(a_.z, in_slope); a_.w = bfo_lrelu(a_.w, in_slope);                          \
        const int v_ = lane + 64 * vs_;                                                              \
        float* dst_ = (vs_ == 1 && lane >= 16) ? strip + G::NROW * G::RAWW : strip + pp_ * G::RAWW + 4 * v_;    \
        *reinterpret_cast<w4_f32x4*>(dst_) = a_;                                                     \
    }
#define TTS_TREAD_JOB(PH, J)                                                                         \
    {                                                                                                \
        const int npr_ = (G::npos(PH) + 1) / 2;                                                      \
        const int pp_ = (J) / npr_, jp_ = (J) % npr_;                                                \
        const float* src_ = strip + pp_ * G::RAWW + tr_off + (G::mlo(PH) + 2 * jp_) * dil;           \
        sx[pp_ / 2][2 * jp_][pp_ % 2] = src_[0];                                                     \
        if (2 * jp_ + 1 < G::npos(PH)) sx[pp_ / 2][2 * jp_ + 1][pp_ % 2] = src_[dil];                \
    }
#define TTS_SXV(M) (w4_f32x2{sv[ol_][0][G::fdiv4((M) - pad_c) - G::vlo(PH_)][((M) - pad_c) - 4 * G::fdiv4((M) - pad_c)],     \
                             sv[ol_][1][G::fdiv4((M) - pad_c) - G::vlo(PH_)][((M) - pad_c) - 4 * G::fdiv4((M) - pad_c)]})
#define TTS_SX(M) (D1 ? TTS_SXV(M) : sx[D1 ? 0 : ol_][D1 ? 0 : (M) - G::mlo(PH_)])
#define TTS_WRITE_JOB(PH, J, WR)                                                                     \
    {                                                                                                \
        const int PH_ = (PH);                                                                        \
        const int ol_ = (J) / G::ngp(PH_), gl_ = (J) % G::ngp(PH_), g_ = G::glo(PH_) + gl_;         \
        w4_f32x2 v2;                                                                                 \
        if (g_ < 6 * NSF) {                                                                          \
            const int s3 = 3 * (g_ / 6), i_ = g_ % 6;                                                \
             \
            if (i_ == 0) v2 = 4.f * TTS_SX(s3) + (TTS_SX(s3 + 4) - 5.f * TTS_SX(s3 + 2));           \
            else if (i_ == 1) {                                                                      \
                ta[ol_] = TTS_SX(s3 + 4) - 4.f * TTS_SX(s3 + 2);                                     \
                tb[ol_] = TTS_SX(s3 + 3) - 4.f * TTS_SX(s3 + 1);                                     \
                v2 = ta[ol_] + tb[ol_];                                                              \
            } else if (i_ == 2) v2 = ta[ol_] - tb[ol_];                                              \
            else if (i_ == 3) {                                                                      \
                ta[ol_] = TTS_SX(s3 + 4) - TTS_SX(s3 + 2);                                           \
                tb[ol_] = 2.f * (TTS_SX(s3 + 3) - TTS_SX(s3 + 1));                                   \
                v2 = ta[ol_] + tb[ol_];                                                              \
            } else if (i_ == 4) v2 = ta[ol_] - tb[ol_];                                              \
            else v2 = 4.f * TTS_SX(s3 + 1) + (TTS_SX(s3 + 5 < G::NPOS ? s3 + 5 : s3) - 5.f * TTS_SX(s3 + 3));           \
        } else {                                                                                     \
            v2 = TTS_SX(3 * NSF + (g_ - 6 * NSF));                                                   \
        }                                                                                            \
        (WR)[2 * ((ol_ * 2 * NGPM + gl_) * NTUP)] = v2;                                              \
    }

    const float4* sB = smem4 + kk * NGPM * NTUP + wn * 32 + l31;
    w4_f32x2* sW = reinterpret_cast<w4_f32x2*>(smem4 + skk * NGPM * NTUP + lane) + sh;
    float4 bq[2];

    {
#pragma unroll
        for (int st = 0; st < NSTAGE - 1; ++st) {
            const int ph = st % NPH;
            const int xso = min(c_beg + st / NPH, n_chunks - 1) * 8 * NOCT * x_cs;
            if constexpr (D1) {
#pragma unroll
                for (int J = 0; J < G::nljv(ph); ++J) TTS_VLOAD_JOB(ph, J, xso)
#pragma unroll
                for (int J = 0; J < 2 * G::nljv(ph); ++J) TTS_VACT_JOB(ph, J)
            } else {
                if (G::loads_in(ph)) {
#pragma unroll
                    for (int J = 0; J < 2 * G::NROW; ++J) TTS_TLOAD_JOB(J, xso)
#pragma unroll
                    for (int J = 0; J < 2 * G::NROW; ++J) TTS_TSTORE_JOB(J)
                }
#pragma unroll
                for (int J = 0; J < G::nrj(ph); ++J) TTS_TREAD_JOB(ph, J)
            }
            w4_f32x2* wr = sW + 2 * st * G::BUF4;
#pragma unroll
            for (int J = 0; J < G::nwj(ph); ++J) TTS_WRITE_JOB(ph, J, wr)
        }
    }
    __syncthreads();
    bq[0] = sB[0];

    int stage = 0;
    for (int c = c_beg; c < n_chunks; ++c) {
#pragma unroll
        for (int ph = 0; ph < NPH; ++ph) {
            const int tph = (ph + NSTAGE - 1) % NPH;
            const int xso = min(c + (ph + NSTAGE - 1) / NPH, n_chunks - 1) * 8 * NOCT * x_cs;
            const int stage_next = (stage + 1 == NSTAGE) ? 0 : stage + 1;
            const int stage_fill = (stage == 0) ? NSTAGE - 1 : stage - 1;
            w4_f32x2* wr = sW + 2 * stage_fill * G::BUF4;
            const float4* rd = sB + stage * G::BUF4;
            const int sn = (c + 1 < n_chunks || ph + 1 < NPH) ? stage_next : stage;
#pragma unroll
            for (int gs = 0; gs < NOCT * G::ngq(ph); ++gs) {
                const int ol = gs / G::ngq(ph), gl = gs % G::ngq(ph);
                const int qs = G::WSHARE ? ol % PF : gs % PF;
                const w4_f32x4 a4 = aq[qs];
                if (!G::WSHARE || gl == G::ngq(ph) - 1) {
                    aq[qs] = __builtin_bit_cast(w4_f32x4, bfo_ld16(wrs, wv, wso, 0));
                    wso = min(wso + wstep, wlast);
                }
                if (gl >= G::ngp(ph)) continue;
                const int r = ol * G::ngp(ph) + gl;
                const int cur = r & 1, nxt = cur ^ 1;
                const int plane = G::plane(G::glo(ph) + gl);
                if (r + 1 < NOCT * G::ngp(ph)) bq[nxt] = rd[(((r + 1) / G::ngp(ph)) * 2 * NGPM + (r + 1) % G::ngp(ph)) * NTUP];
                else if (NSTAGE >= 3) bq[nxt] = sB[sn * G::BUF4];
                __builtin_amdgcn_sched_barrier(0);
                const float bv[4] = {bq[cur].x, bq[cur].y, bq[cur].z, bq[cur].w};
#pragma unroll
                for (int m = 0; m < NM; ++m) {
                    acc[plane] = __builtin_amdgcn_mfma_f32_32x32x2f32(a4[m], bv[m], acc[plane], 0, 0, 0);
                    const int t = r * NM + m;
                    if constexpr (D1) {
                        if (t < G::nljv(tph)) TTS_VLOAD_JOB(tph, t, xso)
                        if (t >= G::DAV && t - G::DAV < 2 * G::nljv(tph)) TTS_VACT_JOB(tph, t - G::DAV)
                        if (t >= G::tw0v(tph) && (t - G::tw0v(tph)) % G::wsv(tph) == 0 &&
                            (t - G::tw0v(tph)) / G::wsv(tph) < G::nwj(tph))
                            TTS_WRITE_JOB(tph, (t - G::tw0v(tph)) / G::wsv(tph), wr)
                    } else {
                        if (G::loads_in(tph) && t < 2 * G::NROW) TTS_TLOAD_JOB(t, xso)
                        if (G::loads_in(tph) && t >= G::DAT && t < G::DAT + 2 * G::NROW) TTS_TSTORE_JOB(t - G::DAT)
                        if (t >= G::tr_r0(tph) && t - G::tr_r0(tph) < G::nrj(tph)) TTS_TREAD_JOB(tph, t - G::tr_r0(tph))
                        if (t >= G::tw0t(tph) && (t - G::tw0t(tph)) % G::wst(tph) == 0 && (t - G::tw0t(tph)) / G::wst(tph) < G::nwj(tph))
                            TTS_WRITE_JOB(tph, (t - G::tw0t(tph)) / G::wst(tph), wr)
                    }
                    __builtin_amdgcn_sched_barrier(0);
                }
            }
            __syncthreads();
            if (NSTAGE < 3) bq[0] = sB[sn * G::BUF4];
            else if ((NOCT * G::ngp(ph)) % 2 != 0) bq[0] = bq[1];
            stage = stage_next;
        }
    }
#undef TTS_TLOAD_JOB
#undef TTS_TSTORE_JOB
#undef TTS_TREAD_JOB
#undef TTS_VLOAD_JOB
#undef TTS_VACT_JOB
#undef TTS_VJOB_IDX
#undef TTS_SXV
#undef TTS_SX
#undef TTS_WRITE_JOB

    constexpr int LDS_F = CO_BLK * NT_BLK + CO_BLK;
    constexpr int LPR = NT_BLK / 4;
    static_assert(LPR == 64, "one wave instruction per row");
    float* ep = reinterpret_cast<float*>(smem4);
    float* epb = ep + LDS_F - CO_BLK;
    float* __restrict__ yb = p.y + (int64_t)b * p.y_bs;
    const float* __restrict__ rb = (p.res && !preload) ? p.res + (int64_t)b * p.r_bs : nullptr;
    const int mode = p.mode, relu_out = p.relu_out, Cout = p.Cout;
    const float div = p.div;
    __syncthreads();
    if (tid < CO_BLK) epb[tid] = ep_bias;
#pragma unroll
    for (int r = 0; r < 16; ++r) {
        const int row = wm * 32 + (r & 3) + 8 * (r >> 2) + 4 * kk;
        const float s12 = acc[1][r] + acc[2][r], d12 = acc[1][r] - acc[2][r];
        const float s34 = acc[3][r] + acc[4][r], d34 = acc[3][r] - acc[4][r];
        float y0 = acc[0][r] + s12 + s34;
        float y1 = d12 + 2.f * d34;
        float y2 = s12 + 4.f * s34;
        float y3 = d12 + 8.f * d34 + acc[5][r];
        if constexpr (NSF == 0) { y0 = acc[0][r]; y1 = 0.f; y2 = 0.f; y3 = acc[5][r]; }
        if constexpr (NPL == 8) {
            y1 += acc[6][r];
            y2 += acc[7][r];
        }
        if (pe < ntup_eff) {
            if (dil == 1) {
                *reinterpret_cast<float4*>(ep + row * NT_BLK + col_e) = make_float4(y0, y1, y2, y3);
            } else {
                ep[row * NT_BLK + col_e] = y0;
                ep[row * NT_BLK + col_e + dil] = y1;
                ep[row * NT_BLK + col_e + 2 * dil] = y2;
                ep[row * NT_BLK + col_e + 3 * dil] = y3;
            }
        }
    }
    __syncthreads();
    constexpr int NR = CO_BLK / 4;
    const int col = lane * 4, q = q0 + col;
    if (q >= n_out || col >= nt_eff) return;
    const bool full = q + 3 < n_out;
    if (p.ksplit > 1) {
        float* __restrict__ pb = p.splitk_ws + ((int64_t)ks * p.batch + b) * Cout * p.Nout;
#pragma unroll 4
        for (int it = 0; it < NR; ++it) {
            const int rl = wid + it * 4;
            const int co = co_blk0 + rl;
            if (co >= Cout) continue;
            const float4 a4 = *reinterpret_cast<const float4*>(ep + rl * NT_BLK + col);
            float* yp = pb + (int64_t)co * p.Nout + q;
            if (full && (p.Nout & 3) == 0) {
                *reinterpret_cast<float4*>(yp) = a4;
            } else {
                const float v[4] = {a4.x, a4.y, a4.z, a4.w};
#pragma unroll
                for (int e = 0; e < 4; ++e)
                    if (q + e < n_out) yp[e] = v[e];
            }
        }
        return;
    }
    const float* __restrict__ scale = K == 1 ? p.scale : nullptr;
    const bool plain_act = K != 1 || (relu_out < 2 && scale == nullptr);
    if (plain_act && (preload || (!rb && mode == 0))) {
        const float lo = relu_out == 1 ? 0.f : -__builtin_inff();
        const bool do_div = preload && mode == 2;
#pragma unroll 4
        for (int it = 0; it < NR; ++it) {
            const int rl = wid + it * 4;
            const int co = co_blk0 + rl;
            if (co >= Cout) continue;
            const float bsv = epb[rl];
            const float4 a4 = *reinterpret_cast<const float4*>(ep + rl * NT_BLK + col);
            float v[4] = {fmaxf(a4.x + bsv, lo), fmaxf(a4.y + bsv, lo), fmaxf(a4.z + bsv, lo), fmaxf(a4.w + bsv, lo)};
            if (do_div) {
#pragma unroll
                for (int e = 0; e < 4; ++e) v[e] = v[e] / div;
            }
            float* yp = yb + (int64_t)co * p.y_cs + q;
            if (full) {
                *reinterpret_cast<float4*>(yp) = make_float4(v[0], v[1], v[2], v[3]);
            } else {
#pragma unroll
                for (int e = 0; e < 4; ++e)
                    if (q + e < n_out) yp[e] = v[e];
            }
        }
        return;
    }
    if constexpr (preload) return;
#pragma unroll 2
    for (int it = 0; it < NR; ++it) {
        const int rl = wid + it * 4;
        const int co = co_blk0 + rl;
        if (co >= Cout) continue;
        const float bsv = epb[rl];
        const float4 a4 = *reinterpret_cast<const float4*>(ep + rl * NT_BLK + col);
        float v[4] = {a4.x, a4.y, a4.z, a4.w};
        float* yp = yb + (int64_t)co * p.y_cs + q;
        const float* rp = rb ? rb + (int64_t)co * p.r_cs + q : nullptr;
        float rr4[4] = {0.f, 0.f, 0.f, 0.f}, pp4[4] = {0.f, 0.f, 0.f, 0.f};
        if (full) {
            if (rp) { const float4 t = *reinterpret_cast<const float4*>(rp); rr4[0] = t.x; rr4[1] = t.y; rr4[2] = t.z; rr4[3] = t.w; }
            if (mode != 0) { const float4 t = *reinterpret_cast<const float4*>(yp); pp4[0] = t.x; pp4[1] = t.y; pp4[2] = t.z; pp4[3] = t.w; }
        } else {
#pragma unroll
            for (int e = 0; e < 4; ++e)
                if (q + e < n_out) {
                    if (rp) rr4[e] = rp[e];
                    if (mode != 0) pp4[e] = yp[e];
                }
        }
        const float scv = (K == 1 && scale) ? scale[co] : 1.f;
#pragma unroll
        for (int e = 0; e < 4; ++e) {
            float x = v[e] + bsv;
            if constexpr (K == 1) {
                if (relu_out == 2) x = 0.5f * x * (1.0f + erff(x * 0.70710678118654752440f));
                x = x * scv;
            }
            x += rr4[e];
            if (relu_out == 1) x = fmaxf(x, 0.f);
            if constexpr (K == 1) { if (relu_out == 3) x = tanhf(x); }
            if (mode == 1) x = pp4[e] + x;
            else if (mode == 2) x = (pp4[e] + x) / div;
            v[e] = x;
        }
        if (full) {
            *reinterpret_cast<float4*>(yp) = make_float4(v[0], v[1], v[2], v[3]);
        } else {
#pragma unroll
            for (int e = 0; e < 4; ++e)
                if (q + e < n_out) yp[e] = v[e];
        }
    }
}

template <int K, int NOCT, int NSTAGE, int EPI, int LP>
static int32_t launch_wino4_epi(const ConvParams& p, hipStream_t stream) {
    using G = Wino4Geo<K, NOCT, NSTAGE, EPI>;
    constexpr size_t ring = (size_t)G::NSTAGE * G::BUF4 * sizeof(float4);
    constexpr size_t epi = ((size_t)G::CO_BLK * G::NT_BLK + G::CO_BLK) * sizeof(float);
    constexpr size_t strip = LP == 2 ? (size_t)G::RAW_BYTES : 0;
    constexpr size_t lds = ring + strip > epi ? ring + strip : epi;
    static_assert(lds <= 80 * 1024, "two blocks per CU");
    static std::atomic<uint64_t> lds_done{0};
    const auto kern = conv1d_wino4_f32<K, NOCT, NSTAGE, EPI, LP>;
    TTS_CHECK_HIP(lds_opt_in((const void*)kern, (int)lds, lds_done));
    const int nt = wino4_tile(p.dil, G::NTUP);
    ConvParams q = p;
    q.ksplit = EPI == 0 ? wino4_ksplit(p) : 1;
    const int64_t n_tiles = (int64_t)((p.Nout + nt - 1) / nt) * p.batch;
    const int64_t n_blocks = ((n_tiles + 7) / 8) * 8 * (p.CoutP / G::CO_BLK) * q.ksplit;
    TTS_REQUIRE(n_blocks < ((int64_t)1 << 31), "wino4: %lld blocks", (long long)n_blocks);
    dim3 grid((unsigned)n_blocks, 1, 1);
    q.compact = compact_order(p.lens_out, p.batch) ? 1 : 0;
    hipLaunchKernelGGL(kern, grid, dim3(256), lds, stream, q);
    TTS_CHECK_HIP(hipGetLastError());
    if (q.ksplit > 1) return launch_splitk_reduce(q, stream);
    return 0;
}

template <int K, int NOCT, int NSTAGE>
static int32_t launch_wino4_cfg(const ConvParams& p, hipStream_t stream) {
    if (p.dil == 1) {
        if (p.res != nullptr && wino4_ksplit(p) == 1) return launch_wino4_epi<K, NOCT, NSTAGE, 3, 1>(p, stream);
        return launch_wino4_epi<K, NOCT, NSTAGE, 0, 1>(p, stream);
    }
    return launch_wino4_epi<K, NOCT, 2, 0, 2>(p, stream);
}

int32_t launch_wino4(const ConvParams& p, hipStream_t stream) {
    if (p.K == 1) return launch_wino4_epi<1, 4, 2, 0, 1>(p, stream);
    if (p.K == 3) return launch_wino4_cfg<3, 2, 3>(p, stream);
    if (p.K == 7) return launch_wino4_cfg<7, 1, 2>(p, stream);
    if (p.K == 11) return launch_wino4_cfg<11, 1, 3>(p, stream);
    set_error("wino4: kernel size %d not built (1, 3, 7, 11)", p.K);
    return TTSAMD_EINVAL;
}

int wino4_block_outputs(int dil) { return wino4_tile(dil, 64); }

int wino4_ksplit(const ConvParams& p) {
    const int bo = wino4_block_outputs(p.dil);
    const int64_t blocks = (int64_t)((p.Nout + bo - 1) / bo) * (p.CoutP / 64) * p.batch;
    constexpr int sk_blocks = 192, sk_target = 224;
    if (blocks >= sk_blocks || p.splitk_ws == nullptr) return 1;
    const int n_chunks = p.Cin / (p.K == 1 ? 32 : (p.K == 3 ? 16 : 8));
    const int64_t per = (int64_t)p.batch * p.Cout * p.Nout;
    int64_t ks = std::min<int64_t>((sk_target + blocks - 1) / blocks, n_chunks / 8);
    ks = std::min<int64_t>(ks, p.splitk_floats / std::max<int64_t>(per, 1));
    return ks >= 2 ? (int)ks : 1;
}

int wino4_groups(int k) { return k == 3 ? 6 : (k == 7 ? 16 : 24); }

void wino4_filter_groups(const float* g, int k, float* o) {
    const int nsf = k == 3 ? 1 : (k == 7 ? 2 : 4);
    for (int s = 0; s < nsf; ++s) {
        const double g0 = g[3 * s], g1 = 3 * s + 1 < k ? g[3 * s + 1] : 0.0, g2 = 3 * s + 2 < k ? g[3 * s + 2] : 0.0;
        o[6 * s] = (float)(g0 / 4);
        o[6 * s + 1] = (float)(-(g0 + g1 + g2) / 6);
        o[6 * s + 2] = (float)(-(g0 - g1 + g2) / 6);
        o[6 * s + 3] = (float)(g0 / 24 + g1 / 12 + g2 / 6);
        o[6 * s + 4] = (float)(g0 / 24 - g1 / 12 + g2 / 6);
        o[6 * s + 5] = (float)g2;
    }
    if (k == 7)
        for (int j = 0; j < 4; ++j) o[12 + j] = g[6];
}

void pack_wino4_weight(const float* w, int cout, int cin, int k, float* out) {
    const int ng = wino4_groups(k);
    std::vector<float> u((size_t)cout * cin * ng);
    for (int64_t i = 0; i < (int64_t)cout * cin; ++i) wino4_filter_groups(w + i * k, k, u.data() + i * ng);
    pack_conv_weight(u.data(), cout, cin, ng, out);
}

}
```

tts-arabic-pytorch_amd/ttsamd/lib.py:

```python
import ctypes as C
import os

_HERE = os.path.dirname(os.path.abspath(__file__))
LIB_PATH = os.environ.get('TTSAMD_LIB') or os.path.join(_HERE, 'lib', 'libttsamd.so')


class TtsAmdError(RuntimeError):
    pass


class Tensor(C.Structure):
    _fields_ = [('name', C.c_char_p), ('data', C.POINTER(C.c_float)), ('ndim', C.c_int32),
                ('shape', C.c_int64 * 4)]


class HifiGanCfg(C.Structure):
    _fields_ = [('num_mels', C.c_int32), ('upsample_initial_channel', C.c_int32), ('n_ups', C.c_int32),
                ('upsample_rates', C.c_int32 * 8), ('upsample_kernel_sizes', C.c_int32 * 8),
                ('n_kernels', C.c_int32), ('resblock_kernel_sizes', C.c_int32 * 8),
                ('n_dilations', C.c_int32), ('resblock_dilations', (C.c_int32 * 8) * 8), ('resblock', C.c_int32)]


class FastPitchCfg(C.Structure):
    _fields_ = [(n, C.c_int32) for n in (
        'n_mel_channels', 'n_symbols', 'padding_idx', 'd_model',
        'in_fft_n_layers', 'in_fft_n_heads', 'in_fft_d_head', 'in_fft_kernel', 'in_fft_filter',
        'out_fft_n_layers', 'out_fft_n_heads', 'out_fft_d_head', 'out_fft_kernel', 'out_fft_filter',
        'dur_kernel', 'dur_filter', 'dur_n_layers',
        'pitch_kernel', 'pitch_filter', 'pitch_n_layers', 'pitch_emb_kernel',
        'energy_conditioning', 'energy_kernel', 'energy_filter', 'energy_n_layers', 'energy_emb_kernel',
        'n_speakers')] + [('speaker_emb_weight', C.c_float)]


class Tacotron2Cfg(C.Structure):
    _fields_ = [(n, C.c_int32) for n in (
        'n_symbol', 'num_speakers', 'speaker_embedding_dim', 'symbol_embedding_dim', 'encoder_embedding_dim',
        'encoder_n_convolution', 'encoder_kernel_size', 'n_mels', 'prenet_dim', 'attention_rnn_dim',
        'decoder_rnn_dim', 'attention_hidden_dim', 'attention_location_n_filter',
        'attention_location_kernel_size', 'postnet_n_convolution', 'postnet_kernel_size',
        'postnet_embedding_dim')] + [('gate_threshold', C.c_float), ('decoder_early_stopping', C.c_int32)]


class TaggerCfg(C.Structure):
    _fields_ = [('n_vocab', C.c_int32), ('emb_dim', C.c_int32), ('n_lstm', C.c_int32), ('lstm_hidden', C.c_int32 * 4),
                ('hard_sigmoid', C.c_int32), ('bn_after_lstm0', C.c_int32), ('bn_eps', C.c_float),
                ('n_dense', C.c_int32), ('dense_dim', C.c_int32 * 4)]


_P, _I32, _I64, _F = C.c_void_p, C.c_int32, C.c_int64, C.c_float
SYMBOLS = {
    'ttsamd_last_error': (C.c_char_p, []),
    'ttsamd_version': (_I32, []),
    'ttsamd_set_option': (_I32, [C.c_char_p, C.c_char_p]),
    'ttsamd_get_option': (_I32, [C.c_char_p, C.c_char_p, _I32]),
    'ttsamd_option_name': (C.c_char_p, [_I32]),
    'ttsamd_options_check': (_I32, []),
    'ttsamd_device_ok': (_I32, []),
    'ttsamd_hifigan_create': (_I32, [C.POINTER(Tensor), _I32, C.POINTER(HifiGanCfg), C.POINTER(_P)]),
    'ttsamd_hifigan_destroy': (_I32, [_P]),
    'ttsamd_hifigan_workspace_bytes': (_I64, [_P, _I32, _I32]),
    'ttsamd_hifigan_forward': (_I32, [_P, _P, _P, _I32, _I32, _P, _P, _I64, _P]),
    'ttsamd_fastpitch_create': (_I32, [C.POINTER(Tensor), _I32, C.POINTER(FastPitchCfg), C.POINTER(_P)]),
    'ttsamd_fastpitch_destroy': (_I32, [_P]),
    'ttsamd_fastpitch_encode_workspace_bytes': (_I64, [_P, _I32, _I32]),
    'ttsamd_fastpitch_decode_workspace_bytes': (_I64, [_P, _I32, _I32]),
    'ttsamd_fastpitch_encode': (_I32, [_P, _P, _I32, _I32, _I32, _F, _P, _P, _P, _F, _F, _F,
                                       _P, _P, _P, _P, _P, _P, _P, _I64, _P]),
    'ttsamd_length_regulate': (_I32, [_P, _P, _I32, _I32, _I32, _I32, _P, _P, _P]),
    'ttsamd_fastpitch_decode': (_I32, [_P, _P, _P, _I32, _I32, _P, _P, _I64, _P]),
    'ttsamd_fastpitch_set_batch_mode': (_I32, [_P, _I32]),
    'ttsamd_denoiser_create': (_I32, [C.POINTER(_P)]),
    'ttsamd_denoiser_destroy': (_I32, [_P]),
    'ttsamd_denoiser_workspace_bytes': (_I64, [_I32, _I32]),
    'ttsamd_denoiser_bias_spec': (_I32, [_P, _P, _P, _I32, _P, _P, _I64, _P]),
    'ttsamd_denoise': (_I32, [_P, _P, _I64, _P, _I32, _I32, _P, _F, _P, _I64, _P]),
    'ttsamd_vocos_create': (_I32, [C.POINTER(Tensor), _I32, _I32, _I32, _I32, _I32, C.POINTER(_P)]),
    'ttsamd_vocos_destroy': (_I32, [_P]),
    'ttsamd_vocos_workspace_bytes': (_I64, [_P, _I32, _I32]),
    'ttsamd_vocos_bias_vec': (_I32, [_P, _P, _P, _I64, _P]),
    'ttsamd_vocos_forward': (_I32, [_P, _P, _P, _I32, _I32, _F, _P, _P, _P, _I64, _P]),
    'ttsamd_vocos_set_padding': (_I32, [_P, _I32]),
    'ttsamd_melspec_create': (_I32, [_P, _I32, _I32, _I32, _I32, _I32, _F, C.POINTER(_P)]),
    'ttsamd_melspec_destroy': (_I32, [_P]),
    'ttsamd_melspec_forward': (_I32, [_P, _P, _I64, _P, _I32, _I32, _P, _P, _P]),
    'ttsamd_cepstral_series': (_I32, [_P, _P, _I32, _I32, _I32, _I32, _I32, _I32, _F, _P, _P, _P]),
    'ttsamd_cepstral_series_from_power': (_I32, [_P, _P, _I32, _I32, _I32, _I32, _I32, _I32, C.c_double, C.c_double, _F, _P, _P]),
    'ttsamd_series_summary': (_I32, [_P, _P, _I32, _I32, _I32, _P, _P, _P]),
    'ttsamd_dtw_workspace_bytes': (_I64, [_I32, _I32, _I32, _I32]),
    'ttsamd_dtw': (_I32, [_P, _P, _P, _P, _I32, _I32, _I32, _I32, _I32, _I32, _P, _P, _P, _P, _I64, _P]),
    'ttsamd_dtw_aligned_mae': (_I32, [_P, _P, _I32, _I32, _I32, _P, _P, _P, _P]),
    'ttsamd_tacotron2_create': (_I32, [C.POINTER(Tensor), _I32, C.POINTER(Tacotron2Cfg), C.POINTER(_P)]),
    'ttsamd_tacotron2_destroy': (_I32, [_P]),
    'ttsamd_tacotron2_workspace_bytes': (_I64, [_P, _I32, _I32, _I32]),
    'ttsamd_tacotron2_infer': (_I32, [_P, _P, _P, _P, _I32, _I32, _I32, _I64, _P, _P, _P, _P,
                                      C.POINTER(_I32), _P, _I64, _P]),
    'ttsamd_tagger_create': (_I32, [C.POINTER(Tensor), _I32, C.POINTER(TaggerCfg), C.POINTER(_P)]),
    'ttsamd_tagger_destroy': (_I32, [_P]),
    'ttsamd_tagger_workspace_bytes': (_I64, [_P, _I32, _I32]),
    'ttsamd_tagger_forward': (_I32, [_P, _P, _I32, _I32, _P, _P, _I64, _P]),
    'ttsamd_conv1d_packed_floats': (_I64, [_I32, _I32, _I32]),
    'ttsamd_conv1d': (_I32, [_P, _P, _P, _P, _I32, _I32, _I32, _I32, _I32, _I32, _F, _I32, _P, _P, _P]),
    'ttsamd_conv1d_ex': (_I32, [_P, _P, _P, _P, _P, _I32, _I32, _I32, _I32, _I32, _I32, _F, _I32, _I32, _F, _P, _P, _P]),
    'ttsamd_resblock_pair_packed_floats': (_I64, [_I32, _I32, _I32]),
    'ttsamd_resblock_pair': (_I32, [_P, _P, _P, _P, _P, _P, _I32, _I32, _I32, _P, _I32, _I32, _I32, _I32, _F, _F, _I32, _P, _I64, _P]),
    'ttsamd_resblock2_packed_floats': (_I64, [_I32, _I32, _I32]),
    'ttsamd_resblock2': (_I32, [_P, _P, _P, _P, _P, _P, _I32, _I32, _I32, _I32, _P, _I32, _I32, _I32, _I32, _F, _F, _I32, _P, _I64, _P]),
    'ttsamd_bfo_pack': (_I32, [_P, _I32, _I32, _I32, _F, _P, _P]),
    'ttsamd_bfo_unpack': (_I32, [_P, _I32, _I32, _I32, _F, _P, _P]),
    'ttsamd_bfo_weight_elems': (_I64, [_I32, _I32, _I32, _I32]),
    'ttsamd_bfo_pack_weight': (_I32, [_P, _I32, _I32, _I32, _I32, _P]),
    'ttsamd_bfo_conv1d': (_I32, [_P, _P, _P, _P, _P, _P, _I32, _I32, _I32, _I32, _I32, _I32, _I32, _I32, _I32, _F, _F, _F, _P, _P, _P, _P]),
    'ttsamd_bfo_resblock_pair': (_I32, [_P, _P, _P, _P, _P, _P, _P, _I32, _I32, _I32, _I32, _I32, _I32, _I32, _F, _F, _F, _F, _P, _P]),
    'ttsamd_bfo_resblock_chain': (_I32, [_P, _P, _P, _P, _P, _P, _P, _P, _I32, _I32, _I32, _I32, _I32, _F, _F, _F, _F, _P, _P, _I32]),
    'ttsamd_bfo_conv_post': (_I32, [_P, _P, _P, _P, _I32, _I32, _I32, _I32, _P, _I64, _P]),
    'ttsamd_bfo3_pack': (_I32, [_P, _I32, _I32, _I32, _F, _P, _P]),
    'ttsamd_bfo3_unpack': (_I32, [_P, _I32, _I32, _I32, _F, _P, _P]),
    'ttsamd_bfo3_weight_elems': (_I64, [_I32, _I32, _I32, _I32]),
    'ttsamd_bfo3_pack_weight': (_I32, [_P, _I32, _I32, _I32, _I32, _P]),
    'ttsamd_bfo3_conv1d': (_I32, [_P, _P, _P, _P, _P, _P, _I32, _I32, _I32, _I32, _I32, _I32, _I32, _I32, _I32, _F, _F, _F, _P, _P, _P, _P]),
    'ttsamd_bfo3_resblock_pair': (_I32, [_P, _P, _P, _P, _P, _P, _P, _I32, _I32, _I32, _I32, _I32, _I32, _I32, _F, _F, _F, _F, _P, _P]),
    'ttsamd_bfo3_resblock_chain': (_I32, [_P, _P, _P, _P, _P, _P, _P, _P, _I32, _I32, _I32, _I32, _I32, _F, _F, _F, _F, _P, _P]),
    'ttsamd_bfo3_conv_post': (_I32, [_P, _P, _P, _P, _I32, _I32, _I32, _I32, _P, _I64, _P]),
    'ttsamd_set_precision': (_I32, [_I32]),
    'ttsamd_get_precision': (_I32, []),
    'ttsamd_dp_unique_id': (_I32, [_P]),
    'ttsamd_dp_init': (_I32, [_I32, _I32, _P, C.POINTER(_P)]),
    'ttsamd_dp_destroy': (_I32, [_P]),
    'ttsamd_dp_rank': (_I32, [_P]),
    'ttsamd_dp_world': (_I32, [_P]),
    'ttsamd_dp_broadcast': (_I32, [_P, _P, _I64, _I32, _P]),
    'ttsamd_dp_broadcast_weights': (_I32, [_P, _I32, _P, _I32, _P]),
    'ttsamd_dp_allgather': (_I32, [_P, _P, _P, _I64, _P]),
    'ttsamd_dp_pack_audio': (_I32, [_P, _I64, _P, _I32, _I64, _P, _P]),
    'ttsamd_dp_gather_audio': (_I32, [_P, _P, _P, C.POINTER(_I64), C.POINTER(_I64), _I32, _P]),
    'ttsamd_profile_enable': (_I32, [_I32]),
    'ttsamd_profile_read': (_I32, [C.POINTER(C.c_double)]),
}

_lib = None
ABI_VERSION = 8


def load():
    global _lib
    if _lib is not None:
        return _lib
    if not os.path.exists(LIB_PATH):
        raise TtsAmdError(f'{LIB_PATH} is missing: build it with `make -C tts-arabic-pytorch_amd/csrc` '
                          '(hipcc --offload-arch=gfx950); there is no CPU/PyTorch fallback')
    import torch
    lib = C.CDLL(LIB_PATH)
    for name, (res, args) in SYMBOLS.items():
        fn = getattr(lib, name)
        fn.restype, fn.argtypes = res, args
    got = lib.ttsamd_version()
    if got != ABI_VERSION:
        raise TtsAmdError(f'{LIB_PATH} was built from another revision of include/ttsamd.h (library ABI {got}, this binding '
                          f'{ABI_VERSION}): rebuild it with `make -C tts-arabic-pytorch_amd/csrc`')
    if lib.ttsamd_options_check() != 0:
        msg = lib.ttsamd_last_error()
        raise TtsAmdError(f'bad routing option in the environment: {msg.decode() if msg else "?"}')
    _lib = lib
    return lib


def set_option(name, value):
    v = None if value is None else str(value).encode()
    check(load().ttsamd_set_option(name.encode(), v), f'set_option({name}={value})')


def get_option(name):
    buf = C.create_string_buffer(64)
    check(load().ttsamd_get_option(name.encode(), buf, 64), f'get_option({name})')
    return buf.value.decode() or None


def option_names():
    lib, out, i = load(), [], 0
    while True:
        n = lib.ttsamd_option_name(i)
        if not n:
            return out
        out.append(n.decode())
        i += 1


class options:

    def __init__(self, **kv):
        self.kv = kv

    def __enter__(self):
        self.old = {k: get_option(k) for k in self.kv}
        for k, v in self.kv.items():
            set_option(k, v)
        return self

    def __exit__(self, *a):
        for k, v in self.old.items():
            set_option(k, v)


def check(rc, what):
    if rc != 0:
        msg = load().ttsamd_last_error()
        raise TtsAmdError(f'{what} failed ({rc}): {msg.decode() if msg else "?"}')


def make_tensors(state_dict):
    import numpy as np
    keep, items = [], []
    for name, v in state_dict.items():
        if hasattr(v, 'detach'):
            if not v.is_floating_point():
                continue
            v = v.detach().cpu().float().numpy()
        a = np.ascontiguousarray(v, dtype=np.float32)
        if a.ndim > 4:
            continue
        t = Tensor()
        nb = name.encode()
        t.name = nb
        t.data = a.ctypes.data_as(C.POINTER(C.c_float))
        t.ndim = a.ndim
        for i, s in enumerate(a.shape):
            t.shape[i] = s
        keep += [a, nb]
        items.append(t)
    arr = (Tensor * len(items))(*items)
    return arr, keep
```

Baseline: 69.57 million.

## Make Winograd-4 conv kernel persistent with epilogue overlapped with next tile prologue

Restructures the wino4 conv kernel into a persistent loop where each block walks multiple output tiles, overlapping the previous tile's epilogue stores with the next tile's input and weight prefetch. The grid can be capped to a multiple of the CU count behind a new W4_WALK option, and launch statistics counters are added. This aims to cut per-block launch and prologue cost and tail effects, but adds register pressure and complexity. The kernel restructure also changes the non-walk path and the weight prefetch wraparound.

```diff
diff --git a/include/ttsamd.h b/include/ttsamd.h
--- a/include/ttsamd.h
+++ b/include/ttsamd.h
@@ -88,6 +88,7 @@
 const char* ttsamd_option_name(int32_t index);
 int32_t ttsamd_options_check(void);
 int32_t ttsamd_device_ok(void);
+int32_t ttsamd_wino4_launch_stats(int64_t* out4);
 
 
 int32_t ttsamd_hifigan_create(const ttsamd_tensor* weights, int32_t n_weights,
diff --git a/tts-arabic-pytorch_amd/csrc/api.hip b/tts-arabic-pytorch_amd/csrc/api.hip
--- a/tts-arabic-pytorch_amd/csrc/api.hip
+++ b/tts-arabic-pytorch_amd/csrc/api.hip
@@ -248,6 +248,12 @@
     return std::string(prop.gcnArchName).rfind("gfx950", 0) == 0 ? 1 : 0;
 }
 
+int32_t ttsamd_wino4_launch_stats(int64_t* out4) {
+    TTS_REQUIRE(out4 != nullptr, "wino4_launch_stats: null argument");
+    wino4_launch_stats(out4);
+    return 0;
+}
+
 int32_t ttsamd_hifigan_create(const ttsamd_tensor* weights, int32_t n, const ttsamd_hifigan_cfg* cfg, void** handle) {
     HifiGan* h = nullptr;
     const int32_t rc = hifigan_create(weights, n, cfg, &h);
diff --git a/tts-arabic-pytorch_amd/csrc/common.hpp b/tts-arabic-pytorch_amd/csrc/common.hpp
--- a/tts-arabic-pytorch_amd/csrc/common.hpp
+++ b/tts-arabic-pytorch_amd/csrc/common.hpp
@@ -54,6 +54,7 @@
     X(WINO, 0, 0, 1)                                              \
     X(WINO2, 0, 0, 31)             \
     X(WINO4, 0, 0, 31)             \
+    X(W4_WALK, 0, 0, 1)            \
     X(FUSED_PAIR, 0, 0, 1)                   \
     X(FUSED2, 0, 0, 1)                                           \
     X(FUSED2_MASK, 1, 0, 0x1ff)               \
@@ -184,6 +185,7 @@
 int wino4_ksplit(const ConvParams& p);
 int32_t launch_splitk_reduce(const ConvParams& q, hipStream_t stream);
 int32_t launch_wino4(const ConvParams& p, hipStream_t stream);
+void wino4_launch_stats(int64_t* out4);
 void wino4_filter_groups(const float* g, int k, float* o);
 void pack_wino4_weight(const float* w, int cout, int cin, int k, float* out);
 void pack_conv_weight(const float* w, int cout, int cin, int k, float* out);
diff --git a/tts-arabic-pytorch_amd/csrc/conv_wino4.hip b/tts-arabic-pytorch_amd/csrc/conv_wino4.hip
--- a/tts-arabic-pytorch_amd/csrc/conv_wino4.hip
+++ b/tts-arabic-pytorch_amd/csrc/conv_wino4.hip
@@ -2,6 +2,7 @@
 #include <cstring>
 
 #include <algorithm>
+#include <atomic>
 #include <vector>
 
 #include "conv_mfma_common.hpp"
@@ -91,93 +92,73 @@
     const int nt_eff = wino4_tile(dil, NTUP), ntup_eff = nt_eff / 4;
     const int tiles_y = p.CoutP / CO_BLK;
     const int per_tile = tiles_y * p.ksplit;
-    const unsigned sidx = blockIdx.x, xcd = sidx & 7u, u = sidx >> 3;
-    const int yk = (int)(u % (unsigned)per_tile);
-    const unsigned gt = (u / (unsigned)per_tile) * 8u + xcd;
     const int n_tiles_x = (p.Nout + nt_eff - 1) / nt_eff;
-    int b = (int)(gt / (unsigned)n_tiles_x);
-    int q0 = (int)(gt % (unsigned)n_tiles_x) * nt_eff;
-    if (p.compact) {
-        int tile = 0;
-        if (!live_tile(p.lens_out, p.len_out_mul, p.Nout, nt_eff, p.batch, gt, b, tile)) return;
-        b = __builtin_amdgcn_readfirstlane(b);
-        q0 = __builtin_amdgcn_readfirstlane(tile) * nt_eff;
-    } else if (b >= p.batch) {
-        return;
-    }
+    const unsigned n_total = (((unsigned)n_tiles_x * (unsigned)p.batch + 7u) / 8u) * 8u * (unsigned)per_tile;
+    const unsigned gstep = gridDim.x, xcd = blockIdx.x & 7u;
+    const int yk = (int)((blockIdx.x >> 3) % (unsigned)per_tile);
+    unsigned s_nx = blockIdx.x;
+    int b_nx_ = 0, q0_nx_ = 0, n_out_nx_ = 0, in_len_nx_ = 0;
+    auto find_tile = [&]() -> bool {
+        for (; s_nx < n_total; s_nx += gstep) {
+            const unsigned gt = ((s_nx >> 3) / (unsigned)per_tile) * 8u + xcd;
+            int bb = (int)(gt / (unsigned)n_tiles_x);
+            int qq = (int)(gt % (unsigned)n_tiles_x) * nt_eff;
+            if (p.compact) {
+                int tile = 0;
+                if (__builtin_amdgcn_readfirstlane((int)live_tile(p.lens_out, p.len_out_mul, p.Nout, nt_eff, p.batch, gt, bb, tile)) == 0) return false;
+                bb = __builtin_amdgcn_readfirstlane(bb);
+                qq = __builtin_amdgcn_readfirstlane(tile) * nt_eff;
+            } else if (bb >= p.batch) {
+                return false;
+            }
+            int no = p.Nout;
+            if (p.lens_out) no = min(no, (int)p.lens_out[bb] * p.len_out_mul);
+            if (qq >= no) continue;
+            int il = p.Lin;
+            if (p.lens_in) il = min(il, (int)p.lens_in[bb] * p.len_in_mul);
+            b_nx_ = __builtin_amdgcn_readfirstlane(bb); q0_nx_ = __builtin_amdgcn_readfirstlane(qq);
+            n_out_nx_ = __builtin_amdgcn_readfirstlane(no); in_len_nx_ = __builtin_amdgcn_readfirstlane(il);
+            return true;
+        }
+        return false;
+    };
+    bool have_nx = __builtin_amdgcn_readfirstlane((int)find_tile()) != 0;
+    if (!have_nx) return;
     const int tid = threadIdx.x, lane = tid & 63, wid = tid >> 6;
     const int wm = wid / WN, wn = wid % WN;
     const int ks = yk / tiles_y;
     const int co_blk0 = (yk - ks * tiles_y) * CO_BLK;
-    int n_out = p.Nout;
-    if (p.lens_out) n_out = min(n_out, (int)p.lens_out[b] * p.len_out_mul);
-    if (q0 >= n_out) return;
-    int in_len = p.Lin;
-    if (p.lens_in) in_len = min(in_len, (int)p.lens_in[b] * p.len_in_mul);
 
     const int x_cs = p.x_cs, CoutP = p.CoutP;
     const int chunks_all = p.Cin / (8 * NOCT);
     const int c_beg = (int)((int64_t)ks * chunks_all / p.ksplit), n_chunks = (int)((int64_t)(ks + 1) * chunks_all / p.ksplit);
     const int n_groups = (p.Cin / 8) * G::NGW;
-    const float* __restrict__ xb = p.x + (int64_t)b * p.x_bs;
     const float in_slope = p.in_slope;
-
-    float ep_bias = 0.f;
-    if (tid < CO_BLK && p.bias) ep_bias = p.bias[min(co_blk0 + tid, p.Cout - 1)];
 
     const int kk = lane >> 5, l31 = lane & 31;
     const int pe = wn * 32 + l31;
     const int col_e = dil == 1 ? 4 * pe : (pe / dil) * 4 * dil + pe % dil;
     f32x16 acc[NPL];
-#pragma unroll
-    for (int g = 0; g < NPL; ++g)
-#pragma unroll
-        for (int r = 0; r < 16; ++r) acc[g][r] = 0.f;
     constexpr bool preload = EPI == 3;
-    if constexpr (preload) {
-        const int wm_s = __builtin_amdgcn_readfirstlane(wm);
-        const int row0 = co_blk0 + wm_s * 32;
-        const int qv = q0 + col_e;
-        const int voff = (qv < n_out ? qv : 0) * 4;
-        {
-            const int r_cs = p.r_cs;
-            const bfo_i4 rs = bfo_rsrc(p.res + (int64_t)b * p.r_bs, (unsigned)p.Cout * (unsigned)r_cs * 4u);
-            const int vk = 4 * kk * r_cs * 4;
-#pragma unroll
-            for (int r = 0; r < 16; ++r) {
-                const w4_f32x4 t = __builtin_bit_cast(w4_f32x4, bfo_ld16(rs, voff + vk, (row0 + (r & 3) + 8 * (r >> 2)) * r_cs * 4, 0));
-                acc[0][r] = t.x; acc[6][r] = t.y; acc[7][r] = t.z; acc[5][r] = t.w;
-            }
-        }
-        if (p.mode != 0) {
-            const int y_cs_ = p.y_cs;
-            const bfo_i4 ys = bfo_rsrc(p.y + (int64_t)b * p.y_bs, (unsigned)p.Cout * (unsigned)y_cs_ * 4u);
-            const int vk = 4 * kk * y_cs_ * 4;
-#pragma unroll
-            for (int r = 0; r < 16; ++r) {
-                const w4_f32x4 t = __builtin_bit_cast(w4_f32x4, bfo_ld16(ys, voff + vk, (row0 + (r & 3) + 8 * (r >> 2)) * y_cs_ * 4, 0));
-                acc[0][r] += t.x; acc[6][r] += t.y; acc[7][r] += t.z; acc[5][r] += t.w;
-            }
-        }
-    }
+    const int mode = p.mode;
 
     const bfo_i4 wrs = bfo_rsrc(K == 1 ? p.w : p.w_wino4, (unsigned)n_groups * 2u * (unsigned)CoutP * 16u);
     const int wv = (kk * CoutP + co_blk0 + wm * 32 + l31) * 16;
-    const int wstep = 2 * CoutP * 16, wlast = (n_groups - 1) * wstep;
-    int wso = c_beg * NOCT * G::NGW * wstep;
+    const int wstep = 2 * CoutP * 16;
+    const int wbeg = c_beg * NOCT * G::NGW * wstep, wlast = (n_chunks * NOCT * G::NGW - 1) * wstep;
+    int wso = wbeg;
     w4_f32x4 aq[PF];
 #pragma unroll
     for (int g = 0; g < PF; ++g) {
         aq[g] = __builtin_bit_cast(w4_f32x4, bfo_ld16(wrs, wv, wso, 0));
-        wso = min(wso + wstep, wlast);
+        wso = wso + wstep > wlast ? wbeg : wso + wstep;
     }
 
     const int sh = __builtin_amdgcn_readfirstlane((tid >> 7) & 1), skk = __builtin_amdgcn_readfirstlane((tid >> 6) & 1);
     w4_f32x2 sx[D1 ? 1 : NOCT][D1 ? 1 : NPOSP];
     w4_f32x4 sv[D1 ? NOCT : 1][2][D1 ? G::NVP : 1];
     w4_f32x2 ta[NOCT], tb[NOCT];
-    const int spe = min(lane, ntup_eff - 1);
-    const int xw0 = (q0 + 4 * lane) * 4;
+    int xw0 = 0;
     constexpr int pad_c = (K - 1) / 2;
     const int ch_off = (4 * sh + skk) * x_cs;
 
@@ -202,8 +183,7 @@
         }                                                                                            \
     }
     float* const strip = reinterpret_cast<float*>(smem4 + NSTAGE * G::BUF4) + wid * (G::NROW * G::RAWW + 4);
-    const int tr_a = (q0 - pad_c * dil) & ~3;
-    const int tr_off = q0 + (dil == 1 ? 4 * spe : (spe / dil) * 4 * dil + spe % dil) - pad_c * dil - tr_a;
+    int tr_off = 0;
     w4_f32x4 rv[TR ? G::NROW : 1][2];
 #define TTS_TLOAD_JOB(J, XSO)                                                                        \
     {                                                                                                \
@@ -263,20 +243,188 @@
     w4_f32x2* sW = reinterpret_cast<w4_f32x2*>(smem4 + skk * NGPM * NTUP + lane) + sh;
     float4 bq[2];
 
+    constexpr int LDS_F = CO_BLK * NT_BLK + CO_BLK;
+    constexpr int LPR = NT_BLK / 4;
+    static_assert(LPR == 64, "one wave instruction per row");
+    float* ep = reinterpret_cast<float*>(smem4);
+    float* epb = ep + LDS_F - CO_BLK;
+    const int relu_out = p.relu_out, Cout = p.Cout;
+    const float div = p.div;
+    bool have_pv = false;
+    int b_pv_ = 0, q0_pv_ = 0, n_out_pv_ = 0;
+
+    for (;;) {
+    if (have_nx) {
+        int lane_o = lane;
+        asm volatile("" : "+v"(lane_o));
+        const int spe_o = min(lane_o, ntup_eff - 1);
+        const int b_nx = __builtin_amdgcn_readfirstlane(b_nx_), q0_nx = __builtin_amdgcn_readfirstlane(q0_nx_);
+        const int n_out_nx = __builtin_amdgcn_readfirstlane(n_out_nx_), in_len_nx = __builtin_amdgcn_readfirstlane(in_len_nx_);
+        const float* __restrict__ xb = p.x + (int64_t)b_nx * p.x_bs;
+        const int in_len = in_len_nx;
+        xw0 = (q0_nx + 4 * lane_o) * 4;
+        const int tr_a = (q0_nx - pad_c * dil) & ~3;
+        tr_off = q0_nx + (dil == 1 ? 4 * spe_o : (spe_o / dil) * 4 * dil + spe_o % dil) - pad_c * dil - tr_a;
+        const int xso = c_beg * 8 * NOCT * x_cs;
+        if constexpr (D1) {
+#pragma unroll
+            for (int J = 0; J < G::nljv(0); ++J) TTS_VLOAD_JOB(0, J, xso)
+        } else {
+#pragma unroll
+            for (int J = 0; J < 2 * G::NROW; ++J) TTS_TLOAD_JOB(J, xso)
+        }
+        if constexpr (preload) {
+            const int wm_s = __builtin_amdgcn_readfirstlane(wm);
+            const int row0 = co_blk0 + wm_s * 32;
+            const int kk_o = lane_o >> 5;
+            const int qv = q0_nx + 4 * (wn * 32 + (lane_o & 31));
+            const int voff = (qv < n_out_nx ? qv : 0) * 4;
+            {
+                const int r_cs = p.r_cs;
+                const bfo_i4 rs = bfo_rsrc(p.res + (int64_t)b_nx * p.r_bs, (unsigned)p.Cout * (unsigned)r_cs * 4u);
+                const int vk = 4 * kk_o * r_cs * 4;
+#pragma unroll
+                for (int r = 0; r < 16; ++r) {
+                    const w4_f32x4 t = __builtin_bit_cast(w4_f32x4, bfo_ld16(rs, voff + vk, (row0 + (r & 3) + 8 * (r >> 2)) * r_cs * 4, 0));
+                    acc[1 + (r >> 2)][4 * (r & 3)] = t.x; acc[1 + (r >> 2)][4 * (r & 3) + 1] = t.y;
+                    acc[1 + (r >> 2)][4 * (r & 3) + 2] = t.z; acc[1 + (r >> 2)][4 * (r & 3) + 3] = t.w;
+                }
+            }
+        }
+    }
+    if (have_pv) {
+    const int b_pv = __builtin_amdgcn_readfirstlane(b_pv_), q0_pv = __builtin_amdgcn_readfirstlane(q0_pv_);
+    const int n_out_pv = __builtin_amdgcn_readfirstlane(n_out_pv_);
+    float* __restrict__ yb = p.y + (int64_t)b_pv * p.y_bs;
+    const float* __restrict__ rb = (p.res && !preload) ? p.res + (int64_t)b_pv * p.r_bs : nullptr;
+    const int n_out = n_out_pv;
+    constexpr int NR = CO_BLK / 4;
+    int lane_o = lane;
+    asm volatile("" : "+v"(lane_o));
+    const int wid = __builtin_amdgcn_readfirstlane(tid >> 6);
+    const int col = lane_o * 4, q = q0_pv + col;
+    const float* __restrict__ scale = K == 1 ? p.scale : nullptr;
+    const bool plain_act = K != 1 || (relu_out < 2 && scale == nullptr);
+    const bool full = q + 3 < n_out;
+    if (q >= n_out || col >= nt_eff) {
+    } else if (p.ksplit > 1) {
+        float* __restrict__ pb = p.splitk_ws + ((int64_t)ks * p.batch + b_pv) * Cout * p.Nout;
+#pragma unroll 4
+        for (int it = 0; it < NR; ++it) {
+            const int rl = wid + it * 4;
+            const int co = co_blk0 + rl;
+            if (co >= Cout) continue;
+            const float4 a4 = *reinterpret_cast<const float4*>(ep + rl * NT_BLK + col);
+            float* yp = pb + (int64_t)co * p.Nout + q;
+            if (full && (p.Nout & 3) == 0) {
+                *reinterpret_cast<float4*>(yp) = a4;
+            } else {
+                const float v[4] = {a4.x, a4.y, a4.z, a4.w};
+#pragma unroll
+                for (int e = 0; e < 4; ++e)
+                    if (q + e < n_out) yp[e] = v[e];
+            }
+        }
+    } else if (plain_act && (preload || (!rb && mode == 0))) {
+        const float lo = relu_out == 1 ? 0.f : -__builtin_inff();
+        const bool do_div = preload && mode == 2;
+#pragma unroll 4
+        for (int it = 0; it < NR; ++it) {
+            const int rl = wid + it * 4;
+            const int co = co_blk0 + rl;
+            if (co >= Cout) continue;
+            const float bsv = epb[rl];
+            const float4 a4 = *reinterpret_cast<const float4*>(ep + rl * NT_BLK + col);
+            float v[4] = {fmaxf(a4.x + bsv, lo), fmaxf(a4.y + bsv, lo), fmaxf(a4.z + bsv, lo), fmaxf(a4.w + bsv, lo)};
+            if (do_div) {
+#pragma unroll
+                for (int e = 0; e < 4; ++e) v[e] = v[e] / div;
+            }
+            float* yp = yb + (int64_t)co * p.y_cs + q;
+            if (full) {
+                *reinterpret_cast<float4*>(yp) = make_float4(v[0], v[1], v[2], v[3]);
+            } else {
+#pragma unroll
+                for (int e = 0; e < 4; ++e)
+                    if (q + e < n_out) yp[e] = v[e];
+            }
+        }
+    } else {
+        if constexpr (!preload) {
+#pragma unroll 2
+    for (int it = 0; it < NR; ++it) {
+        const int rl = wid + it * 4;
+        const int co = co_blk0 + rl;
+        if (co >= Cout) continue;
+        const float bsv = epb[rl];
+        const float4 a4 = *reinterpret_cast<const float4*>(ep + rl * NT_BLK + col);
+        float v[4] = {a4.x, a4.y, a4.z, a4.w};
+        float* yp = yb + (int64_t)co * p.y_cs + q;
+        const float* rp = rb ? rb + (int64_t)co * p.r_cs + q : nullptr;
+        float rr4[4] = {0.f, 0.f, 0.f, 0.f}, pp4[4] = {0.f, 0.f, 0.f, 0.f};
+        if (full) {
+            if (rp) { const float4 t = *reinterpret_cast<const float4*>(rp); rr4[0] = t.x; rr4[1] = t.y; rr4[2] = t.z; rr4[3] = t.w; }
+            if (mode != 0) { const float4 t = *reinterpret_cast<const float4*>(yp); pp4[0] = t.x; pp4[1] = t.y; pp4[2] = t.z; pp4[3] = t.w; }
+        } else {
+#pragma unroll
+            for (int e = 0; e < 4; ++e)
+                if (q + e < n_out) {
+                    if (rp) rr4[e] = rp[e];
+                    if (mode != 0) pp4[e] = yp[e];
+                }
+        }
+        const float scv = (K == 1 && scale) ? scale[co] : 1.f;
+#pragma unroll
+        for (int e = 0; e < 4; ++e) {
+            float x = v[e] + bsv;
+            if constexpr (K == 1) {
+                if (relu_out == 2) x = 0.5f * x * (1.0f + erff(x * 0.70710678118654752440f));
+                x = x * scv;
+            }
+            x += rr4[e];
+            if (relu_out == 1) x = fmaxf(x, 0.f);
+            if constexpr (K == 1) { if (relu_out == 3) x = tanhf(x); }
+            if (mode == 1) x = pp4[e] + x;
+            else if (mode == 2) x = (pp4[e] + x) / div;
+            v[e] = x;
+        }
+        if (full) {
+            *reinterpret_cast<float4*>(yp) = make_float4(v[0], v[1], v[2], v[3]);
+        } else {
+#pragma unroll
+            for (int e = 0; e < 4; ++e)
+                if (q + e < n_out) yp[e] = v[e];
+        }
+    }
+        }
+    }
+    }
+    if (!have_nx) break;
+    if (have_pv) __syncthreads();
+    const int b = __builtin_amdgcn_readfirstlane(b_nx_), q0 = __builtin_amdgcn_readfirstlane(q0_nx_);
+    const int n_out = __builtin_amdgcn_readfirstlane(n_out_nx_), in_len = __builtin_amdgcn_readfirstlane(in_len_nx_);
+    const float* __restrict__ xb = p.x + (int64_t)b * p.x_bs;
+    const int tr_a = (q0 - pad_c * dil) & ~3;
+    s_nx += gstep;
+    have_nx = __builtin_amdgcn_readfirstlane((int)find_tile()) != 0;
     {
 #pragma unroll
         for (int st = 0; st < NSTAGE - 1; ++st) {
             const int ph = st % NPH;
             const int xso = min(c_beg + st / NPH, n_chunks - 1) * 8 * NOCT * x_cs;
             if constexpr (D1) {
-#pragma unroll
-                for (int J = 0; J < G::nljv(ph); ++J) TTS_VLOAD_JOB(ph, J, xso)
+                if (st > 0) {
+#pragma unroll
+                    for (int J = 0; J < G::nljv(ph); ++J) TTS_VLOAD_JOB(ph, J, xso)
+                }
 #pragma unroll
                 for (int J = 0; J < 2 * G::nljv(ph); ++J) TTS_VACT_JOB(ph, J)
             } else {
                 if (G::loads_in(ph)) {
-#pragma unroll
-                    for (int J = 0; J < 2 * G::NROW; ++J) TTS_TLOAD_JOB(J, xso)
+                    if (st > 0) {
+#pragma unroll
+                        for (int J = 0; J < 2 * G::NROW; ++J) TTS_TLOAD_JOB(J, xso)
+                    }
 #pragma unroll
                     for (int J = 0; J < 2 * G::NROW; ++J) TTS_TSTORE_JOB(J)
                 }
@@ -286,6 +434,40 @@
             w4_f32x2* wr = sW + 2 * st * G::BUF4;
 #pragma unroll
             for (int J = 0; J < G::nwj(ph); ++J) TTS_WRITE_JOB(ph, J, wr)
+            if (st == 0) {
+                __builtin_amdgcn_sched_barrier(0);
+                if constexpr (preload) {
+#pragma unroll
+                    for (int r = 0; r < 16; ++r) {
+                        const f32x16 c = acc[1 + (r >> 2)];
+                        acc[0][r] = c[4 * (r & 3)]; acc[6][r] = c[4 * (r & 3) + 1]; acc[7][r] = c[4 * (r & 3) + 2]; acc[5][r] = c[4 * (r & 3) + 3];
+                    }
+                    if (mode != 0) {
+                        int lane_o = lane;
+                        asm volatile("" : "+v"(lane_o));
+                        const int wm_s = __builtin_amdgcn_readfirstlane(wm);
+                        const int row0 = co_blk0 + wm_s * 32;
+                        const int qv = q0 + 4 * (wn * 32 + (lane_o & 31));
+                        const int voff = (qv < n_out ? qv : 0) * 4;
+                        const int y_cs_ = p.y_cs;
+                        const bfo_i4 ys = bfo_rsrc(p.y + (int64_t)b * p.y_bs, (unsigned)p.Cout * (unsigned)y_cs_ * 4u);
+                        const int vk = 4 * (lane_o >> 5) * y_cs_ * 4;
+#pragma unroll
+                        for (int r = 0; r < 16; ++r) {
+                            const w4_f32x4 t = __builtin_bit_cast(w4_f32x4, bfo_ld16(ys, voff + vk, (row0 + (r & 3) + 8 * (r >> 2)) * y_cs_ * 4, 0));
+                            acc[0][r] += t.x; acc[6][r] += t.y; acc[7][r] += t.z; acc[5][r] += t.w;
+                        }
+                    }
+                    __builtin_amdgcn_sched_barrier(0);
+                }
+#pragma unroll
+                for (int g = 0; g < NPL; ++g) {
+                    if (preload && (g == 0 || g >= 5)) continue;
+#pragma unroll
+                    for (int r = 0; r < 16; ++r) acc[g][r] = 0.f;
+                }
+                __builtin_amdgcn_sched_barrier(0);
+            }
         }
     }
     __syncthreads();
@@ -309,7 +491,7 @@
                 const w4_f32x4 a4 = aq[qs];
                 if (!G::WSHARE || gl == G::ngq(ph) - 1) {
                     aq[qs] = __builtin_bit_cast(w4_f32x4, bfo_ld16(wrs, wv, wso, 0));
-                    wso = min(wso + wstep, wlast);
+                    wso = wso + wstep > wlast ? wbeg : wso + wstep;
                 }
                 if (gl >= G::ngp(ph)) continue;
                 const int r = ol * G::ngp(ph) + gl;
@@ -345,30 +527,17 @@
             stage = stage_next;
         }
     }
-#undef TTS_TLOAD_JOB
-#undef TTS_TSTORE_JOB
-#undef TTS_TREAD_JOB
-#undef TTS_VLOAD_JOB
-#undef TTS_VACT_JOB
-#undef TTS_VJOB_IDX
-#undef TTS_SXV
-#undef TTS_SX
-#undef TTS_WRITE_JOB
-
-    constexpr int LDS_F = CO_BLK * NT_BLK + CO_BLK;
-    constexpr int LPR = NT_BLK / 4;
-    static_assert(LPR == 64, "one wave instruction per row");
-    float* ep = reinterpret_cast<float*>(smem4);
-    float* epb = ep + LDS_F - CO_BLK;
-    float* __restrict__ yb = p.y + (int64_t)b * p.y_bs;
-    const float* __restrict__ rb = (p.res && !preload) ? p.res + (int64_t)b * p.r_bs : nullptr;
-    const int mode = p.mode, relu_out = p.relu_out, Cout = p.Cout;
-    const float div = p.div;
+
+    int tid_o = tid;
+    asm volatile("" : "+v"(tid_o));
+    float ep_bias = 0.f;
+    if (tid_o < CO_BLK && p.bias) ep_bias = p.bias[min(co_blk0 + tid_o, Cout - 1)];
     __syncthreads();
-    if (tid < CO_BLK) epb[tid] = ep_bias;
+    int ep_col = col_e, ep_row = wm * 32 + 4 * kk;
+    asm volatile("" : "+v"(ep_col), "+v"(ep_row));
 #pragma unroll
     for (int r = 0; r < 16; ++r) {
-        const int row = wm * 32 + (r & 3) + 8 * (r >> 2) + 4 * kk;
+        const int row = ep_row + (r & 3) + 8 * (r >> 2);
         const float s12 = acc[1][r] + acc[2][r], d12 = acc[1][r] - acc[2][r];
         const float s34 = acc[3][r] + acc[4][r], d34 = acc[3][r] - acc[4][r];
         float y0 = acc[0][r] + s12 + s34;
@@ -382,114 +551,50 @@
         }
         if (pe < ntup_eff) {
             if (dil == 1) {
-                *reinterpret_cast<float4*>(ep + row * NT_BLK + col_e) = make_float4(y0, y1, y2, y3);
+                *reinterpret_cast<float4*>(ep + row * NT_BLK + ep_col) = make_float4(y0, y1, y2, y3);
             } else {
-                ep[row * NT_BLK + col_e] = y0;
-                ep[row * NT_BLK + col_e + dil] = y1;
-                ep[row * NT_BLK + col_e + 2 * dil] = y2;
-                ep[row * NT_BLK + col_e + 3 * dil] = y3;
-            }
-        }
-    }
+                ep[row * NT_BLK + ep_col] = y0;
+                ep[row * NT_BLK + ep_col + dil] = y1;
+                ep[row * NT_BLK + ep_col + 2 * dil] = y2;
+                ep[row * NT_BLK + ep_col + 3 * dil] = y3;
+            }
+        }
+    }
+    if (tid_o < CO_BLK) epb[tid_o] = ep_bias;
     __syncthreads();
-    constexpr int NR = CO_BLK / 4;
-    const int col = lane * 4, q = q0 + col;
-    if (q >= n_out || col >= nt_eff) return;
-    const bool full = q + 3 < n_out;
-    if (p.ksplit > 1) {
-        float* __restrict__ pb = p.splitk_ws + ((int64_t)ks * p.batch + b) * Cout * p.Nout;
-#pragma unroll 4
-        for (int it = 0; it < NR; ++it) {
-            const int rl = wid + it * 4;
-            const int co = co_blk0 + rl;
-            if (co >= Cout) continue;
-            const float4 a4 = *reinterpret_cast<const float4*>(ep + rl * NT_BLK + col);
-            float* yp = pb + (int64_t)co * p.Nout + q;
-            if (full && (p.Nout & 3) == 0) {
-                *reinterpret_cast<float4*>(yp) = a4;
-            } else {
-                const float v[4] = {a4.x, a4.y, a4.z, a4.w};
-#pragma unroll
-                for (int e = 0; e < 4; ++e)
-                    if (q + e < n_out) yp[e] = v[e];
-            }
-        }
-        return;
-    }
-    const float* __restrict__ scale = K == 1 ? p.scale : nullptr;
-    const bool plain_act = K != 1 || (relu_out < 2 && scale == nullptr);
-    if (plain_act && (preload || (!rb && mode == 0))) {
-        const float lo = relu_out == 1 ? 0.f : -__builtin_inff();
-        const bool do_div = preload && mode == 2;
-#pragma unroll 4
-        for (int it = 0; it < NR; ++it) {
-            const int rl = wid + it * 4;
-            const int co = co_blk0 + rl;
-            if (co >= Cout) continue;
-            const float bsv = epb[rl];
-            const float4 a4 = *reinterpret_cast<const float4*>(ep + rl * NT_BLK + col);
-            float v[4] = {fmaxf(a4.x + bsv, lo), fmaxf(a4.y + bsv, lo), fmaxf(a4.z + bsv, lo), fmaxf(a4.w + bsv, lo)};
-            if (do_div) {
-#pragma unroll
-                for (int e = 0; e < 4; ++e) v[e] = v[e] / div;
-            }
-            float* yp = yb + (int64_t)co * p.y_cs + q;
-            if (full) {
-                *reinterpret_cast<float4*>(yp) = make_float4(v[0], v[1], v[2], v[3]);
-            } else {
-#pragma unroll
-                for (int e = 0; e < 4; ++e)
-                    if (q + e < n_out) yp[e] = v[e];
-            }
-        }
-        return;
-    }
-    if constexpr (preload) return;
-#pragma unroll 2
-    for (int it = 0; it < NR; ++it) {
-        const int rl = wid + it * 4;
-        const int co = co_blk0 + rl;
-        if (co >= Cout) continue;
-        const float bsv = epb[rl];
-        const float4 a4 = *reinterpret_cast<const float4*>(ep + rl * NT_BLK + col);
-        float v[4] = {a4.x, a4.y, a4.z, a4.w};
-        float* yp = yb + (int64_t)co * p.y_cs + q;
-        const float* rp = rb ? rb + (int64_t)co * p.r_cs + q : nullptr;
-        float rr4[4] = {0.f, 0.f, 0.f, 0.f}, pp4[4] = {0.f, 0.f, 0.f, 0.f};
-        if (full) {
-            if (rp) { const float4 t = *reinterpret_cast<const float4*>(rp); rr4[0] = t.x; rr4[1] = t.y; rr4[2] = t.z; rr4[3] = t.w; }
-            if (mode != 0) { const float4 t = *reinterpret_cast<const float4*>(yp); pp4[0] = t.x; pp4[1] = t.y; pp4[2] = t.z; pp4[3] = t.w; }
-        } else {
-#pragma unroll
-            for (int e = 0; e < 4; ++e)
-                if (q + e < n_out) {
-                    if (rp) rr4[e] = rp[e];
-                    if (mode != 0) pp4[e] = yp[e];
-                }
-        }
-        const float scv = (K == 1 && scale) ? scale[co] : 1.f;
-#pragma unroll
-        for (int e = 0; e < 4; ++e) {
-            float x = v[e] + bsv;
-            if constexpr (K == 1) {
-                if (relu_out == 2) x = 0.5f * x * (1.0f + erff(x * 0.70710678118654752440f));
-                x = x * scv;
-            }
-            x += rr4[e];
-            if (relu_out == 1) x = fmaxf(x, 0.f);
-            if constexpr (K == 1) { if (relu_out == 3) x = tanhf(x); }
-            if (mode == 1) x = pp4[e] + x;
-            else if (mode == 2) x = (pp4[e] + x) / div;
-            v[e] = x;
-        }
-        if (full) {
-            *reinterpret_cast<float4*>(yp) = make_float4(v[0], v[1], v[2], v[3]);
-        } else {
-#pragma unroll
-            for (int e = 0; e < 4; ++e)
-                if (q + e < n_out) yp[e] = v[e];
-        }
-    }
+    have_pv = true;
+    b_pv_ = b; q0_pv_ = q0; n_out_pv_ = n_out;
+    }
+#undef TTS_TLOAD_JOB
+#undef TTS_TSTORE_JOB
+#undef TTS_TREAD_JOB
+#undef TTS_VLOAD_JOB
+#undef TTS_VACT_JOB
+#undef TTS_VJOB_IDX
+#undef TTS_SXV
+#undef TTS_SX
+#undef TTS_WRITE_JOB
+}
+
+constexpr int kW4WalkFactor = 2;
+static std::atomic<int64_t> g_w4_last_grid{0}, g_w4_last_blocks{0}, g_w4_walked{0}, g_w4_split{0};
+
+static hipError_t wino4_cu_count(int& cus) {
+    static std::atomic<int> cached[64];
+    int dev = 0;
+    hipError_t e = hipGetDevice(&dev);
+    if (e != hipSuccess) return e;
+    if (dev >= 0 && dev < 64 && (cus = cached[dev].load(std::memory_order_acquire)) > 0) return hipSuccess;
+    e = hipDeviceGetAttribute(&cus, hipDeviceAttributeMultiprocessorCount, dev);
+    if (e == hipSuccess && dev >= 0 && dev < 64) cached[dev].store(cus, std::memory_order_release);
+    return e;
+}
+
+void wino4_launch_stats(int64_t* out) {
+    out[0] = g_w4_last_grid.load(std::memory_order_relaxed);
+    out[1] = g_w4_last_blocks.load(std::memory_order_relaxed);
+    out[2] = g_w4_walked.load(std::memory_order_relaxed);
+    out[3] = g_w4_split.load(std::memory_order_relaxed);
 }
 
 template <int K, int NOCT, int NSTAGE, int EPI, int LP>
@@ -507,9 +612,22 @@
     ConvParams q = p;
     q.ksplit = EPI == 0 ? wino4_ksplit(p) : 1;
     const int64_t n_tiles = (int64_t)((p.Nout + nt - 1) / nt) * p.batch;
-    const int64_t n_blocks = ((n_tiles + 7) / 8) * 8 * (p.CoutP / G::CO_BLK) * q.ksplit;
+    const int per_tile = (p.CoutP / G::CO_BLK) * q.ksplit;
+    const int64_t n_blocks = ((n_tiles + 7) / 8) * 8 * per_tile;
     TTS_REQUIRE(n_blocks < ((int64_t)1 << 31), "wino4: %lld blocks", (long long)n_blocks);
-    dim3 grid((unsigned)n_blocks, 1, 1);
+    int64_t n_grid = n_blocks;
+    if (q.ksplit == 1 && opt_int(OPT_W4_WALK, 0) != 0) {
+        int cus = 0;
+        TTS_CHECK_HIP(wino4_cu_count(cus));
+        const int64_t unit = 8 * per_tile;
+        const int64_t walk = ((int64_t)2 * cus * kW4WalkFactor + unit - 1) / unit * unit;
+        n_grid = std::min(n_blocks, walk);
+    }
+    g_w4_last_grid.store(n_grid, std::memory_order_relaxed);
+    g_w4_last_blocks.store(n_blocks, std::memory_order_relaxed);
+    if (n_grid < n_blocks) g_w4_walked.fetch_add(1, std::memory_order_relaxed);
+    if (q.ksplit > 1) g_w4_split.fetch_add(1, std::memory_order_relaxed);
+    dim3 grid((unsigned)n_grid, 1, 1);
     q.compact = compact_order(p.lens_out, p.batch) ? 1 : 0;
     hipLaunchKernelGGL(kern, grid, dim3(256), lds, stream, q);
     TTS_CHECK_HIP(hipGetLastError());
diff --git a/tts-arabic-pytorch_amd/ttsamd/lib.py b/tts-arabic-pytorch_amd/ttsamd/lib.py
--- a/tts-arabic-pytorch_amd/ttsamd/lib.py
+++ b/tts-arabic-pytorch_amd/ttsamd/lib.py
@@ -56,6 +56,7 @@
     'ttsamd_option_name': (C.c_char_p, [_I32]),
     'ttsamd_options_check': (_I32, []),
     'ttsamd_device_ok': (_I32, []),
+    'ttsamd_wino4_launch_stats': (_I32, [C.POINTER(_I64)]),
     'ttsamd_hifigan_create': (_I32, [C.POINTER(Tensor), _I32, C.POINTER(HifiGanCfg), C.POINTER(_P)]),
     'ttsamd_hifigan_destroy': (_I32, [_P]),
     'ttsamd_hifigan_workspace_bytes': (_I64, [_P, _I32, _I32]),
@@ -169,6 +170,12 @@
     check(load().ttsamd_set_option(name.encode(), v), f'set_option({name}={value})')
 
 
+def wino4_launch_stats():
+    out = (_I64 * 4)()
+    check(load().ttsamd_wino4_launch_stats(out), 'wino4_launch_stats')
+    return tuple(int(v) for v in out)
+
+
 def get_option(name):
     buf = C.create_string_buffer(64)
     check(load().ttsamd_get_option(name.encode(), buf, 64), f'get_option({name})')
```

After: 68.90 million. No clear change (-1.0%).
